# OPM/opm-autodiff

Measured on AMD Instinct MI355X. Metric: Newton iterations/sec, 1M-cell 3-phase black-oil (assembly + ILU0/BiCGStab solve + update), higher is better.
Workload: dtype f64

## Files before the change

include/opmhip.h:

```cpp
#ifndef OPMHIP_H
#define OPMHIP_H

#ifdef __cplusplus
extern "C" {
#endif

#define OPMHIP_ABI_VERSION 11

typedef struct opmhip_ctx opmhip_ctx;

typedef enum opmhip_status {
    OPMHIP_SUCCESS = 0,
    OPMHIP_ANALYSIS_FAILED = -1,
    OPMHIP_CREATE_PRECONDITIONER_FAILED = -2,
    OPMHIP_UNKNOWN_ERROR = -3,
    OPMHIP_INVALID_ARGUMENT = -4,
    OPMHIP_NOT_READY = -5,
    OPMHIP_DEVICE_ERROR = -6,
    OPMHIP_NO_DEVICE = -7
} opmhip_status;

typedef enum opmhip_reorder {
    OPMHIP_REORDER_LEVEL_SCHEDULING = 1,
    OPMHIP_REORDER_GRAPH_COLORING = 2,
// ... 16 lines not shown

typedef struct opmhip_config {
    int abi_version;
    int device_id;
    int verbosity;
    int maxit;
    double tolerance;
    double ilu_relaxation;
    int relax_mode;
    int reorder;
    int zero_diag_fix;
    int chain_length;
    int spmv_pipe_wgs;
    int preconditioner;
    int cpr_reuse_setup;
    int cpr_async_setup;
    int cpr_amg_ilu_levels;
    int cpr_gather_rows;
    int half_product;
    int pin_host_arrays;
    int fused_reductions;
} opmhip_config;

typedef struct opmhip_result {
    int iterations;
    int converged;
    double reduction;
    double conv_rate;
    double elapsed;
    double it;
    double t_copy;
    double t_factor;
    double t_solve;
    int num_colors;
    int reserved[3];
} opmhip_result;

typedef void (*opmhip_ms_apply_fn)(void* user, const double* h_x, double* h_y);
typedef struct opmhip_wells {
    int num_wells;
    const int* val_pointers;
    const int* Ccols;
    const int* Bcols;
    const double* Cnnzs;
    const double* Dnnzs;
    const double* Bnnzs;
    int num_ms_wells;
    opmhip_ms_apply_fn ms_apply;
    void* ms_user;
    int distributed;
} opmhip_wells;

#define OPMHIP_MS_WELLS_MAX_M 256
#define OPMHIP_MS_WELLS_MAX_KIB 32768
#define OPMHIP_MS_WELLS_TREE_MAX_SEGMENTS 1024
#define OPMHIP_MS_WELLS_DENSE 0
#define OPMHIP_MS_WELLS_TREE 1
#define OPMHIP_MS_WELLS_AUTO 2
typedef struct opmhip_ms_wells {
    int num_ms_wells;
    int dim, dim_wells;
    const int* Mb_pointers;
    const int* Brows;
    const int* block_pointers;
    const int* Bcols;
    const double* Bvals;
    const double* Cvals;
    const int* Dcol_pointers;
    const int* Drows;
    const double* Dvals;
    const int* Dnnz_pointers;
} opmhip_ms_wells;
int opmhip_set_ms_wells(opmhip_ctx* ctx, const opmhip_ms_wells* ms);
int opmhip_get_ms_wells_info(opmhip_ctx* ctx, int info[4]);
int opmhip_set_ms_wells_form(opmhip_ctx* ctx, int form);
int opmhip_get_ms_wells_form_info(opmhip_ctx* ctx, int info[6]);

void opmhip_default_config(opmhip_config* cfg);
int opmhip_create(const opmhip_config* cfg, opmhip_ctx** out);
void opmhip_destroy(opmhip_ctx* ctx);
const char* opmhip_last_error(const opmhip_ctx* ctx);
int opmhip_abi_version(void);
int opmhip_synchronize(opmhip_ctx* ctx);

int opmhip_set_pattern(opmhip_ctx* ctx, int Nb, int nnzb, const int* rows, const int* cols);
int opmhip_set_pattern_dd(opmhip_ctx* ctx, int Nb, int Nghost, int nnzb, const int* rows, const int* cols);

int opmhip_solve_system(opmhip_ctx* ctx, int N, int nnz, int dim, double* vals, const int* rows, const int* cols,
                        const double* b, const opmhip_wells* wells, opmhip_result* res);

int opmhip_get_result(opmhip_ctx* ctx, double* x);

int opmhip_wells_apply_residual(opmhip_ctx* ctx, const opmhip_wells* wells, const double* res_well);
int opmhip_add_well_contributions(opmhip_ctx* ctx, const opmhip_wells* wells);
int opmhip_get_rhs(opmhip_ctx* ctx, double* b);
int opmhip_wells_recover_solution(opmhip_ctx* ctx, const opmhip_wells* wells, const double* res_well, double* xw);

int opmhip_upload_system(opmhip_ctx* ctx, const double* vals, const double* b);
int opmhip_spmv(opmhip_ctx* ctx, const double* x, double* y);
int opmhip_ilu0_factor(opmhip_ctx* ctx, double* lu_out);
int opmhip_ilu0_apply(opmhip_ctx* ctx, const double* d, double* v);
int opmhip_preconditioned_product(opmhip_ctx* ctx, const double* d, double* t, double* z);
int opmhip_set_cpr_weights(opmhip_ctx* ctx, const double* weights);
int opmhip_cpr_recreate(opmhip_ctx* ctx);
int opmhip_get_cpr_weights(opmhip_ctx* ctx, double* weights);

int opmhip_cpr_apply(opmhip_ctx* ctx, const double* d, double* v);
int opmhip_get_ordering(opmhip_ctx* ctx, int* toOrder, int* fromOrder, int* rowsPerColor);
int opmhip_get_ordering_info(opmhip_ctx* ctx, int info[4]);
int opmhip_set_ilu_fillin_level(opmhip_ctx* ctx, int n);
int opmhip_get_ilu_info(opmhip_ctx* ctx, int info[4]);
int opmhip_get_ilu_factors(opmhip_ctx* ctx, int* toOrder, int* lrowptr, int* lcol, int* urowptr, int* ucol, double* L, double* U, double* invD);
int opmhip_get_product_form(opmhip_ctx* ctx, int info[4]);
int opmhip_get_split_assembly(opmhip_ctx* ctx, long long info[4], double* rest, double* matrix);
int opmhip_time_kernel(opmhip_ctx* ctx, int which, int reps, double* ms_per_launch);
int opmhip_cpr_levels(opmhip_ctx* ctx, int* n, int* nnz, int cap);

typedef struct opmhip_fluid {
    int num_pvt, num_sat;
    const double* pvtw;
    const double* density;
    const int* pvdg_ptr;
    const double* pvdg;
    const int* pvto_node_ptr;
    const double* pvto_rs;
    const int* pvto_row_ptr;
    const double* pvto;
    const int* swof_ptr;
    const double* swof;
    const int* sgof_ptr;
    const double* sgof;
    double rock_pref, rock_cr;
    const int* pvtg_node_ptr;
    const double* pvtg_pg;
    const int* pvtg_row_ptr;
    const double* pvtg;
    int num_rock;
    const int* rocktab_ptr;
    const double* rocktab;
    int pc_scaling;
} opmhip_fluid;

#define OPMHIP_SW_PO_SG 0
#define OPMHIP_SW_PO_RS 1
#define OPMHIP_SW_PG_RV 2

int opmhip_set_fluid(opmhip_ctx* ctx, const opmhip_fluid* fluid);

int opmhip_set_static(opmhip_ctx* ctx, const double* trans, const double* area, const double* thpres,
                      const double* poro, const double* volume, const double* depth, const int* pvtnum,
                      const int* satnum, const double* rsmax);

int opmhip_set_problem_extras(opmhip_ctx* ctx, const double* rvmax, const int* rocknum, const double* overburden);

int opmhip_set_composition_change_limits(opmhip_ctx* ctx, const double* drsdt, const int* drsdt_all_cells, const double* drvdt);

int opmhip_set_irreversible_compaction(opmhip_ctx* ctx, int enable);

int opmhip_set_vappars(opmhip_ctx* ctx, int enable, double vap1, double vap2);

int opmhip_set_water_compaction(opmhip_ctx* ctx, int num_tables, const int* num_pressure, const int* num_sw, const double* pressure,
                                const double* sw, const double* pv_mult, const double* trans_mult);
int opmhip_get_max_water_saturation(opmhip_ctx* ctx, double* max_water_saturation);

int opmhip_begin_time_step(opmhip_ctx* ctx, double dt);

// ... 204 lines not shown
```

opm-autodiff_amd/capi.py:

```python
import ctypes as C
import os
import re

import numpy as np

HERE = os.path.dirname(os.path.abspath(__file__))
LIB_PATH = os.environ.get("OPMHIP_LIB", os.path.join(HERE, "libopmhip.so"))
HEADER_PATH = os.path.join(os.path.dirname(HERE), "include", "opmhip.h")

SUCCESS = 0
ANALYSIS_FAILED, CREATE_PRECONDITIONER_FAILED, UNKNOWN_ERROR = -1, -2, -3
INVALID_ARGUMENT, NOT_READY, DEVICE_ERROR, NO_DEVICE = -4, -5, -6, -7
REORDER = {"level_scheduling": 1, "graph_coloring": 2, "graph_coloring_greedy": 3, "line_coloring": 4, "auto": 5, "distance2": 6}
RELAX = {"post_scale": 0, "in_sweep": 1}
PRECONDITIONER = {"ilu0": 0, "cpr_quasiimpes": 1, "cpr": 2, "cpr_trueimpes": 2}


class OpmHipError(RuntimeError):
    def __init__(self, code, msg):
        super().__init__("opmhip status %d: %s" % (code, msg))
        self.code = code


class Config(C.Structure):
# ... 258 lines not shown
    Mbp, blkp, nzp = [0], [0], [0]
    cat = {k: [] for k in ("Brows", "Bcols", "Bvals", "Cvals", "Dcolptr", "Drows", "Dvals")}
    for n, w in enumerate(wells):
        a = {k: np.asarray(w[k]).reshape(-1) for k in cat}
        Mb, nblk, nnz = len(a["Brows"]) - 1, len(a["Bcols"]), len(a["Dvals"])
        if Mb < 1:
            raise ValueError("multisegment well %d: Brows needs Mb + 1 >= 2 entries" % n)
        if a["Brows"][0] != 0 or a["Brows"][-1] != nblk or np.any(np.diff(a["Brows"]) < 0):
            raise ValueError("multisegment well %d: Brows must rise from 0 to the number of blocks (%d)" % (n, nblk))
        if len(a["Bvals"]) != 12 * nblk or len(a["Cvals"]) != 12 * nblk:
            raise ValueError("multisegment well %d: Bvals / Cvals need 12 values per block (%d blocks)" % (n, nblk))
        if len(a["Dcolptr"]) != 4 * Mb + 1:
            raise ValueError("multisegment well %d: Dcolptr needs 4 Mb + 1 = %d entries, has %d" % (n, 4 * Mb + 1, len(a["Dcolptr"])))
        if len(a["Drows"]) != nnz or a["Dcolptr"][0] != 0 or a["Dcolptr"][-1] != nnz or np.any(np.diff(a["Dcolptr"]) < 0):
            raise ValueError("multisegment well %d: Dcolptr must rise from 0 to len(Dvals) = len(Drows)" % n)
        for k in cat:
            cat[k].append(a[k])
        Mbp.append(Mbp[-1] + Mb)
        blkp.append(blkp[-1] + nblk)
        nzp.append(nzp[-1] + nnz)
    keep = [_i32(Mbp), _i32(np.concatenate(cat["Brows"])), _i32(blkp), _i32(np.concatenate(cat["Bcols"])), _f64(np.concatenate(cat["Bvals"])),
            _f64(np.concatenate(cat["Cvals"])), _i32(np.concatenate(cat["Dcolptr"])), _i32(np.concatenate(cat["Drows"])), _f64(np.concatenate(cat["Dvals"])), _i32(nzp)]
    return MsWells(len(wells), 3, 4, *[_ptr(k) for k in keep]), keep


def declared_symbols():
    with open(HEADER_PATH) as f:
        txt = re.sub(r"/\*.*?\*/", "", f.read(), flags=re.S)
    return sorted(set(re.findall(r"\b(opmhip_[a-z0-9_]+)\s*\(", txt)))


_lib = None


def lib():
    global _lib
    if _lib is None:
        if not os.path.exists(LIB_PATH):
            raise OpmHipError(NO_DEVICE, "libopmhip.so not built (%s); run `make -C %s` or "
                              "__graft_entry__.build() - there is no CPU fallback" % (LIB_PATH, HERE))
        L = C.CDLL(LIB_PATH)
        vp, ip, dp = C.c_void_p, C.c_void_p, C.c_void_p
        L.opmhip_abi_version.restype = C.c_int
        L.opmhip_default_config.argtypes = [C.POINTER(Config)]
        L.opmhip_default_config.restype = None
        L.opmhip_create.argtypes = [C.POINTER(Config), C.POINTER(vp)]
        L.opmhip_destroy.argtypes = [vp]
        L.opmhip_destroy.restype = None
        L.opmhip_last_error.argtypes = [vp]
        L.opmhip_last_error.restype = C.c_char_p
        L.opmhip_set_pattern.argtypes = [vp, C.c_int, C.c_int, ip, ip]
        L.opmhip_solve_system.argtypes = [vp, C.c_int, C.c_int, C.c_int, dp, ip, ip, dp, C.POINTER(Wells),
                                          C.POINTER(Result)]
        L.opmhip_get_result.argtypes = [vp, dp]
        L.opmhip_get_rhs.argtypes = [vp, dp]
        L.opmhip_add_well_contributions.argtypes = [vp, C.POINTER(Wells)]
        L.opmhip_wells_apply_residual.argtypes = [vp, C.POINTER(Wells), dp]
        L.opmhip_wells_recover_solution.argtypes = [vp, C.POINTER(Wells), dp, dp]
        L.opmhip_upload_system.argtypes = [vp, dp, dp]
        L.opmhip_spmv.argtypes = [vp, dp, dp]
        L.opmhip_ilu0_factor.argtypes = [vp, dp]
        L.opmhip_ilu0_apply.argtypes = [vp, dp, dp]
        L.opmhip_cpr_apply.argtypes = [vp, dp, dp]
        L.opmhip_preconditioned_product.argtypes = [vp, dp, dp, dp]
        L.opmhip_cpr_recreate.argtypes = [vp]
        L.opmhip_set_cpr_weights.argtypes = [vp, dp]
        L.opmhip_get_cpr_weights.argtypes = [vp, dp]
        L.opmhip_get_ordering.argtypes = [vp, ip, ip, ip]
        L.opmhip_get_ordering_info.argtypes = [vp, C.POINTER(C.c_int * 4)]
        L.opmhip_get_product_form.argtypes = [vp, C.POINTER(C.c_int * 4)]
        L.opmhip_get_split_assembly.argtypes = [vp, C.POINTER(C.c_longlong * 4), dp, dp]
        L.opmhip_set_ilu_fillin_level.argtypes = [vp, C.c_int]
        L.opmhip_get_ilu_info.argtypes = [vp, C.POINTER(C.c_int * 4)]
        L.opmhip_set_ms_wells.argtypes = [vp, C.POINTER(MsWells)]
        L.opmhip_get_ms_wells_info.argtypes = [vp, C.POINTER(C.c_int * 4)]
        L.opmhip_set_ms_wells_form.argtypes = [vp, C.c_int]
        L.opmhip_get_ms_wells_form_info.argtypes = [vp, C.POINTER(C.c_int * 6)]
        L.opmhip_get_ilu_factors.argtypes = [vp, ip, ip, ip, ip, ip, dp, dp, dp]
        L.opmhip_time_kernel.argtypes = [vp, C.c_int, C.c_int, C.POINTER(C.c_double)]
        L.opmhip_cpr_levels.argtypes = [vp, ip, ip, C.c_int]
        L.opmhip_profile_enable.argtypes = [vp, C.c_int]
        L.opmhip_profile_get.argtypes = [vp, C.c_int, C.POINTER(C.c_longlong), C.POINTER(C.c_double)]
        L.opmhip_synchronize.argtypes = [vp]
        L.opmhip_comm_info.argtypes = [vp, ip]
        L.opmhip_comm_selftest.argtypes = [vp, dp]
        L.opmhip_set_vfp_tables.argtypes = [vp, C.POINTER(VfpTables)]
        L.opmhip_vfp_probe.argtypes = [vp, C.c_int, C.c_int, C.c_int, dp, dp, dp, dp, dp, dp, dp]
        _lib = L
    return _lib


def _ptr(a):
    return None if a is None else a.ctypes.data_as(C.c_void_p)


def _f64(a):
    return None if a is None else np.ascontiguousarray(a, dtype=np.float64)


def _i32(a):
    return None if a is None else np.ascontiguousarray(a, dtype=np.int32)


def make_wells(w):
    if not w:
        return None, []
    nstd = int(w.get("numWells", 0))
    if nstd > 0:
        keep = [_i32(w["val_pointers"]), _i32(w["Ccols"]), _i32(w["Bcols"]), _f64(w["Cnnzs"]), _f64(w["Dnnzs"]), _f64(w["Bnnzs"])]
        s = Wells(nstd, *[_ptr(k) for k in keep])
    else:
        keep, s = [], Wells(0)
    nms = int(w.get("numMsWells", 0))
    if nms > 0:
        fn, n = w["ms_apply"], int(w["N"])

        def tramp(_user, hx, hy):
            fn(np.ctypeslib.as_array(hx, shape=(n,)), np.ctypeslib.as_array(hy, shape=(n,)))
        cb = MS_APPLY_FN(tramp)
        keep.append(cb)
        s.num_ms_wells, s.ms_apply = nms, cb
    s.distributed = int(w.get("distributed", 0))
    return s, keep


class HipSolver:

    def __init__(self, verbosity=0, maxit=200, tolerance=1e-2, device_id=0, ilu_relaxation=0.9,
                 relax_mode="post_scale", reorder=None, zero_diag_fix=True, chain_length=0, spmv_pipe_wgs=0,
                 preconditioner="ilu0", cpr_reuse_setup=3, cpr_async_setup=0, cpr_amg_ilu_levels=None, cpr_gather_rows=None, half_product=0, pin_host_arrays=0, fused_reductions=0,
                 ilu_fillin_level=0):
        L = lib()
        cfg = Config()
        L.opmhip_default_config(C.byref(cfg))
        cfg.verbosity, cfg.maxit, cfg.tolerance, cfg.device_id = verbosity, maxit, tolerance, device_id
        cfg.ilu_relaxation = ilu_relaxation
        cfg.relax_mode = RELAX[relax_mode]
        if reorder is not None:
            cfg.reorder = REORDER[reorder]
        cfg.zero_diag_fix = int(zero_diag_fix)
        cfg.chain_length = int(chain_length)
        cfg.spmv_pipe_wgs = int(spmv_pipe_wgs)
        cfg.preconditioner = PRECONDITIONER[preconditioner]
        if cpr_amg_ilu_levels is not None:
            cfg.cpr_amg_ilu_levels = int(cpr_amg_ilu_levels)
        if cpr_gather_rows is not None:
            cfg.cpr_gather_rows = int(cpr_gather_rows)
        cfg.half_product = int(half_product)
        cfg.fused_reductions = int(fused_reductions)
        self._pin = bool(pin_host_arrays)
        cfg.pin_host_arrays = int(pin_host_arrays)
        cfg.cpr_async_setup = int(cpr_async_setup)
        cfg.cpr_reuse_setup = int(cpr_reuse_setup)
        self._h = C.c_void_p()
        rc = L.opmhip_create(C.byref(cfg), C.byref(self._h))
        if rc != SUCCESS:
            raise OpmHipError(rc, L.opmhip_last_error(None).decode())
        self.Nb = self.nnzb = 0
        if ilu_fillin_level:
            self._check(L.opmhip_set_ilu_fillin_level(self._h, int(ilu_fillin_level)))

    def close(self):
        if getattr(self, "_h", None) and self._h.value:
            lib().opmhip_destroy(self._h)
            self._h = C.c_void_p()

# ... 120 lines not shown
    def ordering_info(self):
        info = (C.c_int * 4)()
        self._check(lib().opmhip_get_ordering_info(self._h, C.byref(info)))
        names = {v: k for k, v in REORDER.items()}
        return {"ilu_ordering": names[info[0]], "chain_length": int(info[1]), "colors": int(info[2]), "cpr_amg_ilu_levels": int(info[3])}

    def set_ilu_fillin_level(self, n):
        self._check(lib().opmhip_set_ilu_fillin_level(self._h, int(n)))

    def set_ms_wells(self, wells, form="dense"):
        ms, keep = make_ms_wells(wells)
        if ms:
            self._check(lib().opmhip_set_ms_wells_form(self._h, MS_WELLS_FORMS[form] if isinstance(form, str) else int(form)))
        self._check(lib().opmhip_set_ms_wells(self._h, C.byref(ms) if ms else None))

    def ms_wells_form_info(self):
        info = (C.c_int * 6)()
        self._check(lib().opmhip_get_ms_wells_form_info(self._h, C.byref(info)))
        names = {v: k for k, v in MS_WELLS_FORMS.items()}
        return {"form": names[int(info[0])], "dense": int(info[1]), "tree": int(info[2]), "tree_max_segments": int(info[3]), "tree_max_depth": int(info[4]),
                "tree_kib": int(info[5])}

    def ms_wells_info(self):
        info = (C.c_int * 4)()
        self._check(lib().opmhip_get_ms_wells_info(self._h, C.byref(info)))
        return {"wells": int(info[0]), "max_m": int(info[1]), "kib": int(info[2]), "factorisations": int(info[3])}

    def ilu_info(self):
        info = (C.c_int * 4)()
        self._check(lib().opmhip_get_ilu_info(self._h, C.byref(info)))
        return {"fill_level": int(info[0]), "nl": int(info[1]), "nu": int(info[2]), "levels": int(info[3])}

    def ilu_factors(self, values=True):
        inf = self.ilu_info()
        Nb, nl, nu = self.Nb, inf["nl"], inf["nu"]
        out = {"to": np.empty(Nb, np.int32), "lrowptr": np.empty(Nb + 1, np.int32), "lcol": np.empty(nl, np.int32),
               "urowptr": np.empty(Nb + 1, np.int32), "ucol": np.empty(nu, np.int32)}
        vals = [None, None, None]
        if values:
            vals = [np.empty((nl, 3, 3)), np.empty((nu, 3, 3)), np.empty((Nb, 3, 3))]
            out.update(L=vals[0], U=vals[1], invD=vals[2])
        self._check(lib().opmhip_get_ilu_factors(self._h, *[_ptr(out[k]) for k in ("to", "lrowptr", "lcol", "urowptr", "ucol")],
                                                 *[_ptr(v) for v in vals]))
        return out

    def product_form(self):
        info = (C.c_int * 4)()
        self._check(lib().opmhip_get_product_form(self._h, C.byref(info)))
        return {"half_product": bool(info[0]), "u_is_upper_a": bool(info[1]), "rest_blocks": int(info[2]), "rest_positions": int(info[3])}

    def split_assembly(self, rest=False, matrix=False):
        info = (C.c_longlong * 4)()
        r = np.empty((self.product_form()["rest_blocks"], 3, 3)) if rest else None
        m = np.empty(9 * self.nnzb) if matrix else None
        self._check(lib().opmhip_get_split_assembly(self._h, C.byref(info), _ptr(r), _ptr(m)))
        out = {"on": bool(info[0]), "stale": bool(info[1]), "assemblies": int(info[2]), "gathers": int(info[3])}
        if rest:
            out["rest"] = r
        if matrix:
            out["matrix"] = m
        return out

    PROF = ["spmv", "ilu_apply", "ilu_factor", "vector", "assemble", "iq_update", "convergence", "cpr_amg", "spmv_boundary",
            "halo", "allreduce", "cpr_gather"]

    def profile_enable(self, on=True):
        self._check(lib().opmhip_profile_enable(self._h, int(on)))

    def profile(self):
        out = {}
        for i, name in enumerate(self.PROF):
            n, ms = C.c_longlong(0), C.c_double(0.0)
            self._check(lib().opmhip_profile_get(self._h, i, C.byref(n), C.byref(ms)))
            out[name] = (n.value, ms.value)
        return out

    def cpr_levels(self):
        n, nnz = np.zeros(32, np.int32), np.zeros(32, np.int32)
        L = self._check(lib().opmhip_cpr_levels(self._h, _ptr(n), _ptr(nnz), 32))
        return [int(v) for v in n[:L]], [int(v) for v in nnz[:L]]

    def synchronize(self):
        self._check(lib().opmhip_synchronize(self._h))

    def comm_info(self):
        a = np.zeros(4, np.int32)
        self._check(lib().opmhip_comm_info(self._h, _ptr(a)))
        return {"nranks": int(a[0]), "rank": int(a[1]), "device": int(a[2]), "kind": ["none", "loopback", "rccl"][int(a[3])]}

    def comm_selftest(self):
        a = np.zeros(2)
        self._check(lib().opmhip_comm_selftest(self._h, _ptr(a)))
        return float(a[0]), float(a[1])

    def time_kernel(self, which, reps=20):
        ms = C.c_double()
        self._check(lib().opmhip_time_kernel(self._h, {"spmv": 0, "ilu_apply": 1, "ilu_factor": 2, "vector": 3, "stream_read": 4, "spmv_dot1": 5, "spmv_dot2": 6,
                                                              "rest_product": 7, "rest_product_dot2": 8, "ilu_apply_rowsums": 9}[which],
                                             reps, C.byref(ms)))
        return ms.value


def comm_unique_id():
    L = lib()
    if not getattr(L, "_asm_bound", False):
        _bind_assembly(L)
        L._asm_bound = True
    buf = C.create_string_buffer(128)
    rc = L.opmhip_comm_unique_id(buf)
    if rc != SUCCESS:
        raise OpmHipError(rc, "opmhip_comm_unique_id failed (librccl not loadable?)")
    return buf.raw


def _bind_assembly(L):
    vp = C.c_void_p
    L.opmhip_set_fluid.argtypes = [vp, vp]
    L.opmhip_set_static.argtypes = [vp] + [vp] * 9
    L.opmhip_set_state.argtypes = [vp, vp, vp]
    L.opmhip_get_state.argtypes = [vp, vp, vp]
    L.opmhip_advance_time_level.argtypes = [vp]
    L.opmhip_update_failed.argtypes = [vp]
    L.opmhip_end_time_step.argtypes = [vp, C.c_double]
    L.opmhip_set_drift_compensation.argtypes = [vp, C.c_int, C.c_double]
    L.opmhip_set_source.argtypes = [vp, vp, vp]
    L.opmhip_assemble.argtypes = [vp, C.c_double, C.c_int, vp, vp]
    L.opmhip_get_iq.argtypes = [vp, vp]
    L.opmhip_get_iq_cells.argtypes = [vp, C.c_int, vp, vp]
    L.opmhip_set_source_cells.argtypes = [vp, C.c_int, vp, vp, vp]
    L.opmhip_convergence.argtypes = [vp, C.c_double, C.c_double, vp]
    L.opmhip_update.argtypes = [vp, vp, C.c_double, C.POINTER(C.c_int)]
    L.opmhip_reservoir_averages.argtypes = [vp, vp]
    L.opmhip_set_pattern_dd.argtypes = [vp, C.c_int, C.c_int, C.c_int, vp, vp]
    L.opmhip_comm_unique_id.argtypes = [C.c_char_p]
    L.opmhip_comm_init_rccl.argtypes = [vp, C.c_int, C.c_int, C.c_char_p]
    L.opmhip_comm_init_loopback.argtypes = [vp, C.c_int, C.c_int, C.c_char_p]
    L.opmhip_set_halo.argtypes = [vp, C.c_longlong, C.c_int, vp, vp, vp, vp]
    L.opmhip_set_cell_global_ids.argtypes = [vp, vp]
    L.opmhip_fluid_probe.argtypes = [vp, C.c_int, C.c_int, C.c_int, vp, vp, vp, vp, vp]
    L.opmhip_set_problem_extras.argtypes = [vp, vp, vp, vp]
    L.opmhip_set_pcw.argtypes = [vp, vp]
    L.opmhip_set_endpoint_scaling.argtypes = [vp, vp]
    L.opmhip_set_composition_change_limits.argtypes = [vp, vp, vp, vp]
    L.opmhip_set_irreversible_compaction.argtypes = [vp, C.c_int]
    L.opmhip_begin_time_step.argtypes = [vp, C.c_double]
    L.opmhip_get_trackers.argtypes = [vp, vp, vp, vp, vp]
    L.opmhip_set_vappars.argtypes = [vp, C.c_int, C.c_double, C.c_double]
    L.opmhip_set_water_compaction.argtypes = [vp, C.c_int, vp, vp, vp, vp, vp, vp]
    L.opmhip_get_max_water_saturation.argtypes = [vp, vp]
    L.opmhip_relative_change.argtypes = [vp, C.POINTER(C.c_double)]
    L.opmhip_sat_end_points.argtypes = [vp, C.c_int, vp]
    L.opmhip_sat_probe.argtypes = [vp, C.c_int, vp, C.c_int, vp, vp, vp]
    L.opmhip_gas_probe.argtypes = [vp, C.c_int, C.c_int, vp, vp, vp]
    L.opmhip_iq_fields.argtypes = [vp]
    L.opmhip_set_hysteresis.argtypes = [vp, C.c_int, vp, vp]
    L.opmhip_get_hysteresis.argtypes = [vp, vp, vp, vp, vp]
    L.opmhip_set_hysteresis_params.argtypes = [vp, vp, vp]
    L.opmhip_set_aquifers.argtypes = [vp, C.POINTER(Aquifers)]
    L.opmhip_aquifers_begin_time_step.argtypes = [vp, C.c_double, C.c_double]
    L.opmhip_get_aquifers.argtypes = [vp, vp, vp, vp, vp]
    L.opmhip_get_aquifer_rates.argtypes = [vp, vp]
    L.opmhip_set_std_wells.argtypes = [vp, C.POINTER(StdWells)]
    L.opmhip_std_wells_begin_iteration.argtypes = [vp, C.c_int]
    L.opmhip_std_wells_apply_residual.argtypes = [vp]
    L.opmhip_std_wells_update.argtypes = [vp, C.c_double]
    L.opmhip_get_std_wells.argtypes = [vp, vp, vp, vp]
# ... 375 lines not shown
        n = getattr(self, "_nswperf", 0)
        if (pp is not None and pp.size != n) or (pr is not None and pr.size != 3 * n):
            raise ValueError("set_std_wells_perf_state: array lengths do not fit the %d perforations set" % n)
        self._check(lib().opmhip_set_std_wells_perf_state(self._h, _ptr(pp), _ptr(pr)))

    def std_wells_begin_iteration(self, iteration):
        self._check(lib().opmhip_std_wells_begin_iteration(self._h, int(iteration)))

    def std_wells_apply_residual(self):
        self._check(lib().opmhip_std_wells_apply_residual(self._h))

    def std_wells_update(self, relax=1.0):
        self._check(lib().opmhip_std_wells_update(self._h, float(relax)))

    def get_std_wells(self):
        n = getattr(self, "_nsw", 0)
        x, ctl, rw = np.zeros((n, 4)), np.zeros(n, np.int32), np.zeros((n, 4))
        self._check(lib().opmhip_get_std_wells(self._h, _ptr(x), _ptr(ctl), _ptr(rw)))
        return x, ctl, rw

    def set_std_wells_state(self, x=None, control=None, rate_target=None):
        x, control, rate_target = _f64(x), _i32(control), _f64(rate_target)
        n = getattr(self, "_nsw", 0)
        if (x is not None and x.size != 4 * n) or (control is not None and control.size != n) or (rate_target is not None and rate_target.size != n):
            raise ValueError("set_std_wells_state: array lengths do not fit the %d wells set" % n)
        self._check(lib().opmhip_set_std_wells_state(self._h, _ptr(x), _ptr(control), _ptr(rate_target)))

    def std_wells_blocks(self):
        n, p = getattr(self, "_nsw", 0), getattr(self, "_nswperf", 0)
        out = dict(head=np.zeros(p), D=np.zeros((n, 4, 4)), Dinv=np.zeros((n, 4, 4)), B=np.zeros((p, 4, 3)), C=np.zeros((p, 4, 3)), rates=np.zeros((p, 3, 5)),
                   xw=np.zeros((n, 4)))
        self._check(lib().opmhip_get_std_wells_blocks(self._h, *[_ptr(out[k]) for k in ("head", "D", "Dinv", "B", "C", "rates", "xw")]))
        return out

    def set_source(self, source, dsource=None):
        s, d = _f64(source), _f64(dsource)
        self._check(lib().opmhip_set_source(self._h, _ptr(s), _ptr(d)))

    def set_source_cells(self, cells, source, dsource=None):
        cl, s, d = _i32(cells), _f64(source), _f64(dsource)
        self._check(lib().opmhip_set_source_cells(self._h, len(cl), _ptr(cl), _ptr(s), _ptr(d)))

    def assemble(self, dt, iteration, fetch=True):
        jac = np.empty(9 * self.nnzb) if fetch else None
        res = np.empty(3 * self.Nb) if fetch else None
        self._check(lib().opmhip_assemble(self._h, dt, iteration, _ptr(jac), _ptr(res)))
        return jac, res

    def iq(self):
        nf = self._check(lib().opmhip_iq_fields(self._h))
        out = np.empty(self.Nloc * nf * 4)
        self._check(lib().opmhip_get_iq(self._h, _ptr(out)))
        return out.reshape(self.Nloc, nf, 4)

    def iq_cells(self, cells):
        cl = _i32(cells)
        nf = self._check(lib().opmhip_iq_fields(self._h))
        out = np.empty(len(cl) * nf * 4)
        self._check(lib().opmhip_get_iq_cells(self._h, len(cl), _ptr(cl), _ptr(out)))
        return out.reshape(len(cl), nf, 4)

    def convergence(self, dt, tol_cnv=1e-2):
        out = np.empty(17)
        self._check(lib().opmhip_convergence(self._h, dt, tol_cnv, _ptr(out)))
        return out

    def reservoir_averages(self):
        out = np.empty(5)
        self._check(lib().opmhip_reservoir_averages(self._h, _ptr(out)))
        return out

    def solve_jacobian_system(self, wells=None):
        res = Result()
        ws, keep = make_wells(wells)
        self._check(lib().opmhip_solve_system(self._h, 3 * self.Nb, 9 * self.nnzb, 3, None, None, None, None,
                                              C.byref(ws) if ws else None, C.byref(res)))
        return res

    def update(self, dx=None, relax=1.0):
        dx = _f64(dx)
        n = C.c_int(0)
        self._check(lib().opmhip_update(self._h, _ptr(dx), relax, C.byref(n)))
        return n.value
```

opm-autodiff_amd/csrc/assemble.hip:

```cpp
#include <hip/hip_runtime.h>

#include <cfloat>

#include "device_blocks.hpp"
#include "fluid_device.hpp"

namespace opmhip {

template <class E> __device__ __forceinline__ E wc_eval(const int* __restrict__ d, const double* __restrict__ data, int voff, const E& xv, const E& yv) {
    const int ns = d[1];
    const double* xs = data + d[2];
    const double* ys = data + d[3];
    const int i = seg_right(xs, d[0], val(xv));
    const E alpha = (xv - xs[i]) / (xs[i + 1] - xs[i]);
    const double* v1 = data + voff + (size_t)i * ns;
    const double* v2 = v1 + ns;
    const int j1 = seg_right(ys, ns, val(yv)), j2 = j1;
    const E beta1 = (yv - ys[j1]) / (ys[j1 + 1] - ys[j1]);
    const E beta2 = (yv - ys[j2]) / (ys[j2 + 1] - ys[j2]);
    const E s1 = v1[j1] * (1.0 - beta1) + v1[j1 + 1] * beta1;
    const E s2 = v2[j2] * (1.0 - beta2) + v2[j2 + 1] * beta2;
    return s1 * (1.0 - alpha) + s2 * alpha;
}
template <class E, class DP> __device__ __forceinline__ void cap_pressures(const TablesT<DP>& T, int sr, const E& Sw, const E& Sg, E pC[3]) {
// ... 432 lines not shown
    iq_update_body<EXT>(c0, Nb, T, C, pv, meaning, iq);
}
template <>
__global__ __launch_bounds__(256) IQ_OCC void k_iq_update<false>(int c0, int Nb, Tables T, CellStatic C, const double* __restrict__ pv,
                                                                 const unsigned char* __restrict__ meaning, double* __restrict__ iq) {
    iq_update_body<false>(c0, Nb, T, C, pv, meaning, iq);
}

template <class DP, bool EXT>
__device__ __forceinline__ void newton_update_cell(const TablesT<DP>& T, const CellStatic& C, int c, const double* __restrict__ dx, double relax,
                                                   double* __restrict__ pv, unsigned char* __restrict__ meaning,
                                                   unsigned char* __restrict__ wasSwitched, double* __restrict__ iq,
                                                   int* __restrict__ nswitched) {
    const double dpMaxRel = 0.3, dsMax = 0.2, oscThreshold = 1e-5;
    double x[3] = {pv[(size_t)c * 3], pv[(size_t)c * 3 + 1], pv[(size_t)c * 3 + 2]};
    double u[3] = {dx[(size_t)c * 3], dx[(size_t)c * 3 + 1], dx[(size_t)c * 3 + 2]};
    if (relax != 1.0) { u[0] *= relax; u[1] *= relax; u[2] *= relax; }
    int mng = meaning[c];
    const double deltaSw = u[0];
    double deltaSo = -deltaSw, deltaSg = 0.0;
    if (mng == OPMHIP_SW_PO_SG) { deltaSg = u[2]; deltaSo -= deltaSg; }
    double maxSatDelta = fmax(fabs(deltaSg), fabs(deltaSo));
    maxSatDelta = fmax(maxSatDelta, fabs(deltaSw));
    double satAlpha = 1.0;
    if (maxSatDelta > dsMax) satAlpha = dsMax / maxSatDelta;
    double nx[3];
    {
        double delta = u[0] * satAlpha;
        nx[0] = x[0] - delta;
        delta = u[1];
        if (fabs(delta) > dpMaxRel * x[1]) delta = (delta < 0.0 ? -1.0 : 1.0) * dpMaxRel * x[1];
        nx[1] = x[1] - delta;
        delta = u[2];
        if (mng == OPMHIP_SW_PO_SG) delta *= satAlpha;
        else if (delta > x[2]) delta = x[2];
        nx[2] = x[2] - delta;
    }
    x[0] = nx[0]; x[1] = nx[1]; x[2] = nx[2];
    const int pr = C.pvtnum ? C.pvtnum[c] : 0, sr = C.satnum ? C.satnum[c] : 0;
    const double RsMax = C.rsmax ? C.rsmax[c] : DBL_MAX / 2.0;
    const bool wet = EXT && T.pvt(pr).wg_n > 0;
    const double eps = wasSwitched[c] ? oscThreshold : 0.0;
    bool sw = false;
    const bool vap = EXT && C.maxso;
    auto vap_f = [&](double So_, double par) { return vap ? vappars_factor<double>(So_, emax(So_, C.maxso[c]), par) : 1.0; };
    if (x[0] >= 1.0) {
        x[0] = 1.0; x[2] = 0.0;
        sw = mng != OPMHIP_SW_PO_SG;
        mng = OPMHIP_SW_PO_SG;
    } else if (mng == OPMHIP_SW_PO_SG) {
        const double So = 1.0 - x[0] - x[2];
        if (x[2] < -eps && So > 0.0) {
            mng = OPMHIP_SW_PO_RS;
            x[2] = emin(RsMax, rs_sat_value(T, pr, x[1]) * vap_f(So, C.vap2));
            sw = true;
        } else if (EXT && wet && So < -eps && x[2] > 0.0) {
            double pC[3];
            cell_cap_pressures<DP, EXT>(T, C, c, sr, x[0], x[2], pC);
            const double pg = x[1] + (pC[GAS] - pC[OIL]);
            const double RvMax = C.rvmax ? C.rvmax[c] : DBL_MAX / 2.0;
            mng = OPMHIP_SW_PG_RV;
            x[1] = pg;
            x[2] = emin(RvMax, rv_sat_value(T, pr, pg) * vap_f(So, C.vap1));
            sw = true;
        }
    } else if (!EXT || mng == OPMHIP_SW_PO_RS) {
        const double RsSat = rs_sat_value(T, pr, x[1]) * vap_f(1.0 - x[0], C.vap2);
        if (x[2] > emin(RsMax, RsSat * (1.0 + eps))) { mng = OPMHIP_SW_PO_SG; x[2] = 0.0; sw = true; }
    } else {
        const double RvMax = C.rvmax ? C.rvmax[c] : DBL_MAX / 2.0;
        const double RvSat = rv_sat_value(T, pr, x[1]) * vap_f(0.0, C.vap1);
        if (x[2] > emin(RvMax, RvSat * (1.0 + eps))) {
            double pC[3];
            cell_cap_pressures<DP, EXT>(T, C, c, sr, x[0], 1.0 - x[0], pC);
            mng = OPMHIP_SW_PO_SG;
            x[1] = x[1] + (pC[OIL] - pC[GAS]);
            x[2] = 1.0 - x[0];
            sw = true;
        }
    }
    wasSwitched[c] = sw ? 1 : 0;
    meaning[c] = (unsigned char)mng;
    pv[(size_t)c * 3] = x[0]; pv[(size_t)c * 3 + 1] = x[1]; pv[(size_t)c * 3 + 2] = x[2];
    if (sw) atomicAdd(nswitched, 1);
    Iq<Ad> q;
    update_iq<Ad, DP, EXT>(T, C, c, x, mng, q);
    store_iq<EXT>(iq, C.ncell, c, q);
    store_invb(C.invb, c, q);
}
template <bool EXT>
__device__ __forceinline__ void newton_update_body(int Nb, const Tables& T, const CellStatic& C, const double* __restrict__ dx, double relax,
                                                   double* __restrict__ pv, unsigned char* __restrict__ meaning,
                                                   unsigned char* __restrict__ wasSwitched, double* __restrict__ iq,
                                                   int* __restrict__ nswitched) {
    __shared__ double s_tab[TAB_LDS_DBL];
    const bool inLds = tables_to_lds(T, s_tab);
    const int c = blockIdx.x * blockDim.x + threadIdx.x;
    if (c >= Nb) return;
    if (inLds) newton_update_cell<LdsTab, EXT>(lds_tables(T, s_tab), C, c, dx, relax, pv, meaning, wasSwitched, iq, nswitched);
    else newton_update_cell<GlobalTab, EXT>(T, C, c, dx, relax, pv, meaning, wasSwitched, iq, nswitched);
}
template <bool EXT>
__global__ __launch_bounds__(256) void k_newton_update(int Nb, Tables T, CellStatic C, const double* __restrict__ dx, double relax,
                                                       double* __restrict__ pv, unsigned char* __restrict__ meaning,
                                                       unsigned char* __restrict__ wasSwitched, double* __restrict__ iq,
                                                       int* __restrict__ nswitched) {
    newton_update_body<EXT>(Nb, T, C, dx, relax, pv, meaning, wasSwitched, iq, nswitched);
}
template <>
__global__ __launch_bounds__(256) IQ_OCC void k_newton_update<false>(int Nb, Tables T, CellStatic C, const double* __restrict__ dx, double relax,
                                                                     double* __restrict__ pv, unsigned char* __restrict__ meaning,
                                                                     unsigned char* __restrict__ wasSwitched, double* __restrict__ iq,
                                                                     int* __restrict__ nswitched) {
    newton_update_body<false>(Nb, T, C, dx, relax, pv, meaning, wasSwitched, iq, nswitched);
}

__global__ __launch_bounds__(256) void k_fluid_probe(Tables T, int pr, int sr, int n, const double* __restrict__ p,
                                                     const double* __restrict__ rs, const double* __restrict__ sw,
                                                     const double* __restrict__ sg, double* __restrict__ out) {
    const int i = blockIdx.x * blockDim.x + threadIdx.x;
    if (i >= n) return;
    const PvtRegionDesc& D = T.pvt(pr);
    const SatRegionDesc& Sd = T.sat(sr);
    const GlobalTab B = T.dbl;
    double* o = out + (size_t)i * 8;
    const double pi = p[i], rsi = rs[i];
    o[0] = pvt_invBw(T, D, pi);
    const bool wetg = D.wg_n > 0;
    o[1] = wetg ? tab1<double, GlobalTab>(B + D.wg_xs, B + D.wgs_invB, D.wg_n, pi) : tab1<double, GlobalTab>(B + D.gas_p, B + D.gas_invB, D.gas_n, pi);
    const double RsSat = rs_sat_value(T, pr, pi);
    o[3] = RsSat;
    o[2] = pvt_invBo(T, pr, D, pi, rsi);
    if (rsi >= RsSat) o[6] = o[2] / tab1<double, GlobalTab>(B + D.sat_p, B + D.sat_invBMu, D.sat_n, pi);
    else o[6] = o[2] / tab2<double, GlobalTab>(T, D, D.o_invBMu, rsi, pi);
    const double Swco = B[Sd.swco];
    o[4] = pwlin<double, GlobalTab>(B + Sd.sw_x, B + Sd.pcow, Sd.nw, sw[i]);
    o[5] = pwlin<double, GlobalTab>(B + Sd.so_x, B + Sd.pcgo, Sd.ng, 1.0 - Swco - sg[i]);
    o[7] = o[1] / (wetg ? tab1<double, GlobalTab>(B + D.wg_xs, B + D.wgs_invBMu, D.wg_n, pi) : tab1<double, GlobalTab>(B + D.gas_p, B + D.gas_invBMu, D.gas_n, pi));
}
__global__ __launch_bounds__(256) void k_gas_probe(Tables T, int pr, int n, const double* __restrict__ p, const double* __restrict__ rv,
                                                   double* __restrict__ out) {
    const int i = blockIdx.x * blockDim.x + threadIdx.x;
    if (i >= n) return;
    const PvtRegionDesc& D = T.pvt(pr);
    const GlobalTab B = T.dbl;
    double* o = out + (size_t)i * 3;
    const double pi = p[i], rvi = rv[i];
    o[0] = pvt_invBg(T, pr, D, pi, rvi);
    if (D.wg_n > 0) {
        const double RvSat = rv_sat_value(T, pr, pi);
        o[2] = RvSat;
        if (rvi >= RvSat) o[1] = o[0] / tab1<double, GlobalTab>(B + D.wg_xs, B + D.wgs_invBMu, D.wg_n, pi);
        else o[1] = o[0] / tab2wg<double, GlobalTab>(T, D, D.wg_invBMu, pi, rvi);
    } else {
        o[1] = o[0] / tab1<double, GlobalTab>(B + D.gas_p, B + D.gas_invBMu, D.gas_n, pi);
        o[2] = 0.0;
    }
}
int launch_gas_probe(opmhip_ctx* c, int pr, int n, const double* d_in, double* d_out) {
    hipLaunchKernelGGL(k_gas_probe, dim3((n + 255) / 256), dim3(256), 0, c->stream, tables_of(c), pr, n, d_in, d_in + n, d_out);
    return OPMHIP_SUCCESS;
}
__global__ __launch_bounds__(256) void k_sat_probe(Tables T, int sr, int cfg, const double* __restrict__ eps, int n, const double* __restrict__ sw,
                                                   const double* __restrict__ sg, double* __restrict__ out) {
    const int i = blockIdx.x * blockDim.x + threadIdx.x;
    if (i >= n) return;
    const SatRegionDesc& Sd = T.sat(sr);
// ... 299 lines not shown
    double a[10];
    for (int i = 0; i < 10; ++i) a[i] = (i >= 3 && i < 6) ? -DBL_MAX : 0.0;
    if (c < Nb) {
        const double pvValue = C.poro[c] * C.volume[c];
        const int comp[3] = {EQ_WATER, EQ_OIL, EQ_GAS};
        for (int ph = 0; ph < 3; ++ph) {
            const int e = comp[ph];
            a[6 + e] = 1.0 / C.invb[(size_t)c * 3 + ph];
            const double R2 = resid[(size_t)c * 3 + e];
            a[e] = R2;
            a[3 + e] = fabs(R2) / pvValue;
        }
        a[9] = pvValue;
    }
    const int lane = threadIdx.x & 63, wv = threadIdx.x >> 6;
    for (int i = 0; i < 10; ++i) {
        double v = a[i];
        for (int o = 32; o > 0; o >>= 1) {
            const double w = __shfl_down(v, o, 64);
            v = (i >= 3 && i < 6) ? fmax(v, w) : v + w;
        }
        if (lane == 0) sh[i][wv] = v;
    }
    __syncthreads();
    if (threadIdx.x < 10) {
        const int i = threadIdx.x;
        double v = sh[i][0];
        for (int w = 1; w < 4; ++w) v = (i >= 3 && i < 6) ? fmax(v, sh[i][w]) : v + sh[i][w];
        part[(size_t)blockIdx.x * 10 + i] = v;
    }
}
__global__ void k_conv_pack(const double* __restrict__ out, double* __restrict__ red) {
    if (threadIdx.x < 3) { red[threadIdx.x] = out[threadIdx.x]; red[3 + threadIdx.x] = out[6 + threadIdx.x]; red[8 + threadIdx.x] = out[3 + threadIdx.x]; }
    if (threadIdx.x == 0) red[6] = out[9];
}
__global__ void k_conv_unpack(const double* __restrict__ red, double global_cells, double* __restrict__ out) {
    if (threadIdx.x < 3) { out[threadIdx.x] = red[threadIdx.x]; out[6 + threadIdx.x] = red[3 + threadIdx.x] / global_cells; out[3 + threadIdx.x] = red[8 + threadIdx.x]; }
    if (threadIdx.x == 0) out[9] = red[6];
}
__global__ __launch_bounds__(256) void k_conv_final1(int nblocks, int Nb, const double* __restrict__ part, double* __restrict__ out) {
    __shared__ double sh[10][256];
    double a[10];
    for (int i = 0; i < 10; ++i) a[i] = (i >= 3 && i < 6) ? -DBL_MAX : 0.0;
    for (int b = threadIdx.x; b < nblocks; b += 256)
        for (int i = 0; i < 10; ++i) {
            const double v = part[(size_t)b * 10 + i];
            a[i] = (i >= 3 && i < 6) ? fmax(a[i], v) : a[i] + v;
        }
    for (int i = 0; i < 10; ++i) sh[i][threadIdx.x] = a[i];
    __syncthreads();
    for (int o = 128; o > 0; o >>= 1) {
        if ((int)threadIdx.x < o)
            for (int i = 0; i < 10; ++i) {
                const double v = sh[i][threadIdx.x + o];
                sh[i][threadIdx.x] = (i >= 3 && i < 6) ? fmax(sh[i][threadIdx.x], v) : sh[i][threadIdx.x] + v;
            }
        __syncthreads();
    }
    if (threadIdx.x < 10) {
        double v = sh[threadIdx.x][0];
        if (threadIdx.x >= 6 && threadIdx.x < 9 && Nb > 0) v /= (double)Nb;
        out[threadIdx.x] = v;
    }
}
__global__ __launch_bounds__(256) void k_conv_pass2(int Nb, CellStatic C, const double* __restrict__ resid, const double* __restrict__ out1,
                                                    double dt, double tol_cnv, double* __restrict__ part) {
    __shared__ double sh[4];
    const int c = blockIdx.x * blockDim.x + threadIdx.x;
    double v = 0.0;
    if (c < Nb) {
        const double pvValue = C.poro[c] * C.volume[c];
        bool violated = false;
        for (int e = 0; e < 3; ++e) {
            const double CNV = resid[(size_t)c * 3 + e] * dt * out1[6 + e] / pvValue;
            violated = violated || (fabs(CNV) > tol_cnv);
        }
        if (violated) v = pvValue;
    }
    for (int o = 32; o > 0; o >>= 1) v += __shfl_down(v, o, 64);
    if ((threadIdx.x & 63) == 0) sh[threadIdx.x >> 6] = v;
    __syncthreads();
    if (threadIdx.x == 0) part[blockIdx.x] = sh[0] + sh[1] + sh[2] + sh[3];
}
__global__ __launch_bounds__(256) void k_conv_final2(int nblocks, const double* __restrict__ part, double* __restrict__ out) {
    __shared__ double sh[256];
    double a = 0.0;
    for (int b = threadIdx.x; b < nblocks; b += 256) a += part[b];
    sh[threadIdx.x] = a;
    __syncthreads();
    for (int o = 128; o > 0; o >>= 1) {
        if ((int)threadIdx.x < o) sh[threadIdx.x] += sh[threadIdx.x + o];
        __syncthreads();
    }
    if (threadIdx.x == 0) out[10] = sh[0];
}

constexpr int RESV_SUMS = 8;
template <bool EXT>
__global__ __launch_bounds__(256) void k_resv_avg_part(int Nb, int ncell, const double* __restrict__ iq, const double* __restrict__ volume,
                                                       double* __restrict__ part) {
    __shared__ double sh[RESV_SUMS][4];
    double a[RESV_SUMS];
    for (int i = 0; i < RESV_SUMS; ++i) a[i] = 0.0;
    for (size_t c = (size_t)blockIdx.x * 256 + threadIdx.x; c < (size_t)Nb; c += (size_t)gridDim.x * 256) {
        const int ci = (int)c;
        const double pv_cell = volume[ci] * iq_at(iq, ncell, Lay<EXT>::F_PORO, ci)[0];
        double hydrocarbon = 1.0;
        hydrocarbon -= iq_at(iq, ncell, F_S + WATER, ci)[0];
        const double po = iq_at(iq, ncell, F_P + OIL, ci)[0], Rs = iq_at(iq, ncell, F_RS, ci)[0];
        const double Rv = EXT ? iq_at(iq, ncell, Lay<EXT>::F_RV, ci)[0] : 0.0;
        const double hpv = pv_cell * hydrocarbon;
        if (hpv > 0.0) { a[0] += hpv; a[1] += po * hpv; a[2] += Rs * hpv; a[3] += Rv * hpv; }
        if (pv_cell > 0.0) { a[4] += pv_cell; a[5] += po * pv_cell; a[6] += Rs * pv_cell; a[7] += Rv * pv_cell; }
    }
    const int lane = threadIdx.x & 63, wv = threadIdx.x >> 6;
    for (int i = 0; i < RESV_SUMS; ++i) {
        double v = a[i];
        for (int o = 32; o > 0; o >>= 1) v += __shfl_down(v, o, 64);
        if (lane == 0) sh[i][wv] = v;
    }
    __syncthreads();
    if (threadIdx.x < RESV_SUMS) {
        const int i = threadIdx.x;
        part[(size_t)blockIdx.x * RESV_SUMS + i] = ((sh[i][0] + sh[i][1]) + sh[i][2]) + sh[i][3];
    }
}
__global__ __launch_bounds__(RESV_FINAL_THREADS) void k_resv_avg_final(int nblocks, const double* __restrict__ part, double* __restrict__ out) {
    __shared__ double sh[RESV_SUMS][RESV_FINAL_THREADS];
    double a[RESV_SUMS];
    for (int i = 0; i < RESV_SUMS; ++i) a[i] = 0.0;
    for (int b = threadIdx.x; b < nblocks; b += RESV_FINAL_THREADS)
        for (int i = 0; i < RESV_SUMS; ++i) a[i] += part[(size_t)b * RESV_SUMS + i];
    for (int i = 0; i < RESV_SUMS; ++i) sh[i][threadIdx.x] = a[i];
    __syncthreads();
    for (int o = RESV_FINAL_THREADS / 2; o > 0; o >>= 1) {
        if ((int)threadIdx.x < o)
            for (int i = 0; i < RESV_SUMS; ++i) sh[i][threadIdx.x] += sh[i][threadIdx.x + o];
        __syncthreads();
    }
    if (threadIdx.x == 0) {
        const double hpv_sum = sh[0][0], pv_sum = sh[4][0];
        const int k = hpv_sum > 0.0 ? 0 : 4;
        const double w = sh[k][0];
        const bool ok = hpv_sum > 0.0 || pv_sum > 0.0;
        out[0] = ok ? sh[k + 1][0] / w : 0.0;
        out[1] = ok ? sh[k + 2][0] / w : 0.0;
        out[2] = ok ? sh[k + 3][0] / w : 0.0;
        out[3] = w;
        out[4] = k == 0 ? 1.0 : 0.0;
        out[5] = pv_sum;
    }
}

__global__ void k_drift_update(int n, const double* __restrict__ resid, double dt, double* __restrict__ drift) {
    const int e = blockIdx.x * blockDim.x + threadIdx.x;
    if (e < n) drift[e] = resid[e] * dt;
}
template <bool EXT>
__global__ __launch_bounds__(256) void k_last_rs_rv(int N, const int* __restrict__ pvtnum, const int* __restrict__ drsdt_all, const double* __restrict__ iq,
                                                    double* __restrict__ lastRs, double* __restrict__ lastRv) {
    const int c = blockIdx.x * blockDim.x + threadIdx.x;
    if (c >= N) return;
    if (lastRs) {
        const int pr = pvtnum ? pvtnum[c] : 0;
        const double Sg = iq_at(iq, N, F_S + GAS, c)[0];
        lastRs[c] = (drsdt_all[pr] || Sg > 1e-7) ? iq_at(iq, N, F_RS, c)[0] : INFINITY;
    }
    if (EXT && lastRv) lastRv[c] = iq_at(iq, N, Lay<EXT>::F_RV, c)[0];
}
__global__ __launch_bounds__(256) void k_set_limits(int N, double dt, const int* __restrict__ pvtnum, const double* __restrict__ drsdt, const double* __restrict__ drvdt,
                                                    const double* __restrict__ lastRs, const double* __restrict__ lastRv, double* __restrict__ rsmax, double* __restrict__ rvmax) {
    const int c = blockIdx.x * blockDim.x + threadIdx.x;
    if (c >= N) return;
    const int pr = pvtnum ? pvtnum[c] : 0;
    if (drsdt) rsmax[c] = (drsdt[pr] < 0.0) ? DBL_MAX / 2.0 : lastRs[c] + drsdt[pr] * dt;
    if (drvdt) rvmax[c] = (drvdt[pr] < 0.0) ? DBL_MAX / 2.0 : lastRv[c] + drvdt[pr] * dt;
}
// ... 143 lines not shown
    hipLaunchKernelGGL(k_aquifer_begin, dim3((Q.nc + 63) / 64), dim3(64), 0, c->stream, Q.nc, c->pat.Nloc, Q.d_pos, c->asmb.d_iq, Q.d_pprev);
}
void launch_aquifer_apply(opmhip_ctx* c) {
    const AquifersDev& Q = c->asmb.aq;
    hipLaunchKernelGGL(k_aquifer_apply, dim3((Q.nd + 63) / 64), dim3(64), 0, c->stream, Q.nd, c->pat.Nloc, aquifer_arrays(Q), Q.d_cpos, Q.d_cptr, Q.d_cconn,
                       c->asmb.d_iq, c->asmb.d_depth, c->asmb.d_source, c->asmb.d_dsource, Q.d_save, Q.d_q);
}
void launch_aquifer_restore(opmhip_ctx* c) {
    const AquifersDev& Q = c->asmb.aq;
    hipLaunchKernelGGL(k_aquifer_restore, dim3((Q.nd + 63) / 64), dim3(64), 0, c->stream, Q.nd, Q.d_cpos, Q.d_save, c->asmb.d_source, c->asmb.d_dsource);
}
void launch_aquifer_end(opmhip_ctx* c, double dt) {
    const AquifersDev& Q = c->asmb.aq;
    hipLaunchKernelGGL(k_aquifer_end, dim3((Q.num + 63) / 64), dim3(64), 0, c->stream, Q.num, dt, Q.d_ptr, Q.d_par, Q.d_q, Q.d_state);
}

__global__ void k_cellvec_to_internal_u8(int Nb, const int* __restrict__ fromOrder, const unsigned char* __restrict__ nat, unsigned char* __restrict__ internal) {
    const int p = blockIdx.x * blockDim.x + threadIdx.x;
    if (p < Nb) internal[p] = nat[fromOrder[p]];
}
__global__ void k_cellvec_to_natural_u8(int Nb, const int* __restrict__ toOrder, const unsigned char* __restrict__ internal, unsigned char* __restrict__ nat) {
    const int i = blockIdx.x * blockDim.x + threadIdx.x;
    if (i < Nb) nat[i] = internal[toOrder[i]];
}
__global__ void k_iq_to_natural(int Nb, int IQS, const int* __restrict__ toOrder, const double* __restrict__ internal, double* __restrict__ nat) {
    const size_t e = (size_t)blockIdx.x * blockDim.x + threadIdx.x;
    if (e >= (size_t)Nb * IQS) return;
    const int i = (int)(e / IQS), q = (int)(e % IQS);
    nat[e] = internal[((size_t)(q >> 2) * Nb + toOrder[i]) * 4 + (q & 3)];
}
__global__ void k_iq_gather(int n, int IQS, int Nb, const int* __restrict__ pos, const double* __restrict__ internal, double* __restrict__ out) {
    const size_t e = (size_t)blockIdx.x * blockDim.x + threadIdx.x;
    if (e >= (size_t)n * IQS) return;
    const int i = (int)(e / IQS), q = (int)(e % IQS);
    out[e] = internal[((size_t)(q >> 2) * Nb + pos[i]) * 4 + (q & 3)];
}
__global__ void k_source_scatter(int n, const int* __restrict__ pos, const double* __restrict__ src, const double* __restrict__ dsrc,
                                 double* __restrict__ source, double* __restrict__ dsource) {
    const int e = blockIdx.x * blockDim.x + threadIdx.x;
    if (e >= n * 12) return;
    const int i = e / 12, q = e % 12;
    if (q < 3) source[(size_t)pos[i] * 3 + q] = src[(size_t)i * 3 + q];
    else if (dsrc) dsource[(size_t)pos[i] * 9 + (q - 3)] = dsrc[(size_t)i * 9 + (q - 3)];
}
__global__ void k_unpermute_blocks(int nnzb, const int* __restrict__ nnzMap, const double* __restrict__ internal, double* __restrict__ nat) {
    const size_t e = (size_t)blockIdx.x * blockDim.x + threadIdx.x;
    if (e >= (size_t)nnzb * BB) return;
    const int k = (int)(e / BB), q = (int)(e % BB);
    nat[(size_t)nnzMap[k] * BB + q] = internal[e];
}

static inline int cdiv(size_t a, size_t b) { return (int)((a + b - 1) / b); }
static CellStatic cells_of(const opmhip_ctx* c) {
    return CellStatic{c->asmb.d_poro, c->asmb.d_volume, c->asmb.d_depth, c->asmb.d_rsmax, c->asmb.d_pvtnum, c->asmb.d_satnum,
                      c->asmb.d_rvmax, c->asmb.d_overburden, c->asmb.d_rocknum, c->asmb.d_pcw, c->asmb.d_minpo, c->asmb.d_maxso, c->asmb.vap1, c->asmb.vap2,
                      c->asmb.d_maxsw, c->asmb.d_sw0, c->asmb.d_wcdesc, c->asmb.d_wcdata, c->asmb.d_eps, c->asmb.epscfg,
                      c->asmb.d_hyst, c->asmb.d_imbnum, c->asmb.d_eps_imb, c->asmb.hyst_model, c->asmb.d_invb, c->pat.Nloc};
}
void launch_hyst_update(opmhip_ctx* c, const double* d_sw_ow, const double* d_sw_go) {
    const int N = c->pat.Nloc;
    hipLaunchKernelGGL(k_hyst_update, dim3((N + 255) / 256), dim3(256), 0, c->stream, N, tables_of(c), cells_of(c), c->asmb.d_iq, c->asmb.d_hyst, d_sw_ow, d_sw_go);
}
#define OPMHIP_LAYOUT(c, call_base, call_ext) do { if ((c)->asmb.ext) { call_ext; } else { call_base; } } while (0)

void launch_iq_update(opmhip_ctx* c) {
    const int Nb = c->pat.Nloc;
    const int ps = prof_begin(c, PROF_IQ_UPDATE);
    OPMHIP_LAYOUT(c,
        hipLaunchKernelGGL(k_iq_update<false>, dim3(cdiv(Nb, 256)), dim3(256), 0, c->stream, 0, Nb, tables_of(c), cells_of(c), c->asmb.d_pv, c->asmb.d_meaning, c->asmb.d_iq),
        hipLaunchKernelGGL(k_iq_update<true>, dim3(cdiv(Nb, 256)), dim3(256), 0, c->stream, 0, Nb, tables_of(c), cells_of(c), c->asmb.d_pv, c->asmb.d_meaning, c->asmb.d_iq));
    prof_end(c, ps);
}
int launch_ghost_refresh(opmhip_ctx* c) {
    if (c->comm.nranks <= 1 || c->pat.Nghost == 0) return OPMHIP_SUCCESS;
    int rc;
    if ((rc = comm_halo_f64(c, c->asmb.d_pv, 3))) return rc;
    if ((rc = comm_halo_u8(c, c->asmb.d_meaning))) return rc;
    const int Nb = c->pat.Nb, Nloc = c->pat.Nloc;
    OPMHIP_LAYOUT(c,
        hipLaunchKernelGGL(k_iq_update<false>, dim3(cdiv(Nloc - Nb, 256)), dim3(256), 0, c->stream, Nb, Nloc, tables_of(c), cells_of(c), c->asmb.d_pv, c->asmb.d_meaning, c->asmb.d_iq),
        hipLaunchKernelGGL(k_iq_update<true>, dim3(cdiv(Nloc - Nb, 256)), dim3(256), 0, c->stream, Nb, Nloc, tables_of(c), cells_of(c), c->asmb.d_pv, c->asmb.d_meaning, c->asmb.d_iq));
    return OPMHIP_SUCCESS;
}
void launch_newton_update(opmhip_ctx* c, const double* d_dx, double relax) {
    const int Nb = c->pat.Nb;
    (void)hipMemsetAsync(c->asmb.d_nswitched, 0, sizeof(int), c->stream);
    const int ps = prof_begin(c, PROF_IQ_UPDATE);
    OPMHIP_LAYOUT(c,
        hipLaunchKernelGGL(k_newton_update<false>, dim3(cdiv(Nb, 256)), dim3(256), 0, c->stream, Nb, tables_of(c), cells_of(c), d_dx, relax, c->asmb.d_pv,
                           c->asmb.d_meaning, c->asmb.d_wasSwitched, c->asmb.d_iq, c->asmb.d_nswitched),
        hipLaunchKernelGGL(k_newton_update<true>, dim3(cdiv(Nb, 256)), dim3(256), 0, c->stream, Nb, tables_of(c), cells_of(c), d_dx, relax, c->asmb.d_pv,
                           c->asmb.d_meaning, c->asmb.d_wasSwitched, c->asmb.d_iq, c->asmb.d_nswitched));
    prof_end(c, ps);
}
void launch_assemble(opmhip_ctx* c, double dt, int iteration) {
    EntryStatic ES{c->asmb.d_trans, c->asmb.d_area, c->asmb.d_thpres};
    const int ps = prof_begin(c, PROF_ASSEMBLE);
    const double* drift = c->asmb.drift_enabled ? c->asmb.d_drift : (const double*)nullptr;
    const int grid = c->asmb.nsched;
    if (iteration == 0 && c->asmb.storage_frozen) iteration = 1;
    const bool split = c->split_asm && c->asmb.split_ok && !c->wells.sw.ma.on;
#define OPMHIP_ASM_LAUNCH(EXT, SPL, WET)                                                                                                                                   \
    hipLaunchKernelGGL((k_assemble<EXT, SPL>), dim3(grid), dim3(ASM_THREADS), 0, c->stream, c->asmb.nsched, reinterpret_cast<const int4*>(c->asmb.d_asm_sched),                \
                       reinterpret_cast<const int2*>(c->asmb.d_asm_desc), WET, ES, cells_of(c), c->asmb.d_iq, c->asmb.d_storageOld, c->asmb.d_source, c->asmb.d_dsource, drift, \
                       c->asmb.max_compensation, dt, iteration, SPL ? c->d_R : c->d_A, c->d_b, c->d_U, c->pat.d_rrowptr, c->pat.d_urowptr)
    if (split) { OPMHIP_LAYOUT(c, OPMHIP_ASM_LAUNCH(false, true, 0), OPMHIP_ASM_LAUNCH(true, true, c->asmb.wet_gas ? 1 : 0)); }
    else { OPMHIP_LAYOUT(c, OPMHIP_ASM_LAUNCH(false, false, 0), OPMHIP_ASM_LAUNCH(true, false, c->asmb.wet_gas ? 1 : 0)); }
#undef OPMHIP_ASM_LAUNCH
    c->A_stale = split;
    if (split) c->split_assemblies++;
    prof_end(c, ps);
}
void launch_last_rs_rv(opmhip_ctx* c) {
    const AsmDev& A = c->asmb;
    const int N = c->pat.Nloc;
    OPMHIP_LAYOUT(c, hipLaunchKernelGGL(k_last_rs_rv<false>, dim3((N + 255) / 256), dim3(256), 0, c->stream, N, A.d_pvtnum, A.d_drsdt_all, A.d_iq, A.drsdt_on ? A.d_lastRs : nullptr, (double*)nullptr),
                  hipLaunchKernelGGL(k_last_rs_rv<true>, dim3((N + 255) / 256), dim3(256), 0, c->stream, N, A.d_pvtnum, A.d_drsdt_all, A.d_iq, A.drsdt_on ? A.d_lastRs : nullptr, A.drvdt_on ? A.d_lastRv : nullptr));
}
void launch_set_limits(opmhip_ctx* c, double dt) {
    const AsmDev& A = c->asmb;
    const int N = c->pat.Nloc;
    hipLaunchKernelGGL(k_set_limits, dim3((N + 255) / 256), dim3(256), 0, c->stream, N, dt, A.d_pvtnum, A.drsdt_on ? A.d_drsdt : nullptr, A.drvdt_on ? A.d_drvdt : nullptr,
                       A.d_lastRs, A.d_lastRv, A.d_rsmax, A.d_rvmax);
}
void launch_min_pressure(opmhip_ctx* c, bool init) {
    const int N = c->pat.Nloc;
    hipLaunchKernelGGL(k_min_pressure, dim3((N + 255) / 256), dim3(256), 0, c->stream, N, init ? 1 : 0, c->asmb.d_iq, c->asmb.d_minpo);
}
void launch_max_oil_saturation(opmhip_ctx* c, bool init) {
    const int N = c->pat.Nloc;
    hipLaunchKernelGGL(k_max_oil_saturation, dim3((N + 255) / 256), dim3(256), 0, c->stream, N, init ? 1 : 0, c->asmb.d_iq, c->asmb.d_maxso);
}
void launch_max_water_saturation(opmhip_ctx* c, bool init) {
    const Pattern& P = c->pat;
    const int N = P.Nloc;
    if (!init && N > 1) hipLaunchKernelGGL(k_copy_entry, dim3(1), dim3(1), 0, c->stream, c->asmb.d_maxsw, P.toOrder[1], P.toOrder[0]);
    hipLaunchKernelGGL(k_max_water_saturation, dim3((N + 255) / 256), dim3(256), 0, c->stream, N, init ? 1 : 0, c->asmb.d_iq, c->asmb.d_maxsw, c->asmb.d_sw0);
}
void launch_storage_old(opmhip_ctx* c) {
    const AsmDev& A = c->asmb;
    const int Nb = c->pat.Nb, N = c->pat.Nloc;
    OPMHIP_LAYOUT(c, hipLaunchKernelGGL(k_storage_old<false>, dim3((Nb + 255) / 256), dim3(256), 0, c->stream, Nb, N, 0, A.d_iq, A.d_storageOld),
                  hipLaunchKernelGGL(k_storage_old<true>, dim3((Nb + 255) / 256), dim3(256), 0, c->stream, Nb, N, A.wet_gas ? 1 : 0, A.d_iq, A.d_storageOld));
}

constexpr int RC_PARTS = 256;
__global__ __launch_bounds__(256) void k_relative_change_part(int Nb, const double* __restrict__ pv, const unsigned char* __restrict__ mg,
                                                              const double* __restrict__ pvOld, const unsigned char* __restrict__ mgOld,
                                                              double* __restrict__ part) {
    __shared__ double sd[256], sn[256];
    double delta = 0.0, denom = 0.0;
    for (int c = blockIdx.x * 256 + threadIdx.x; c < Nb; c += RC_PARTS * 256) {
        const double* a = &pv[(size_t)c * 3];
        const double* b = &pvOld[(size_t)c * 3];
        double sN[3] = {0.0, 0.0, 0.0}, sO[3] = {0.0, 0.0, 0.0};
        double oilN = 1.0, oilO = 1.0;
        sN[WATER] = a[0]; oilN -= sN[WATER];
        if (mg[c] == OPMHIP_SW_PO_SG) { sN[GAS] = a[2]; oilN -= sN[GAS]; }
        sN[OIL] = oilN;
        const double tmp = a[1] - b[1];
        double d = tmp * tmp, q = a[1] * a[1];
        sO[WATER] = b[0]; oilO -= sO[WATER];
        if (mgOld[c] == OPMHIP_SW_PO_SG) { sO[GAS] = b[2]; oilO -= sO[GAS]; }
        sO[OIL] = oilO;
#pragma unroll
        for (int ph = 0; ph < 3; ++ph) {
            const double t = sN[ph] - sO[ph];
            d += t * t;
            q += sN[ph] * sN[ph];
        }
        delta += d;
        denom += q;
    }
    sd[threadIdx.x] = delta; sn[threadIdx.x] = denom;
    __syncthreads();
    for (int h = 128; h > 0; h >>= 1) {
        if ((int)threadIdx.x < h) { sd[threadIdx.x] += sd[threadIdx.x + h]; sn[threadIdx.x] += sn[threadIdx.x + h]; }
        __syncthreads();
    }
    if (threadIdx.x == 0) { part[blockIdx.x] = sd[0]; part[RC_PARTS + blockIdx.x] = sn[0]; }
}
__global__ __launch_bounds__(64) void k_relative_change_final(const double* __restrict__ part, double* __restrict__ out) {
    if (threadIdx.x != 0) return;
    double d = 0.0, q = 0.0;
    for (int i = 0; i < RC_PARTS; ++i) { d += part[i]; q += part[RC_PARTS + i]; }
    out[0] = d; out[1] = q;
}
int launch_relative_change(opmhip_ctx* c) {
    const AsmDev& A = c->asmb;
    double* part = A.d_rc;
    double* out = A.d_rc + 2 * RC_PARTS;
    hipLaunchKernelGGL(k_relative_change_part, dim3(RC_PARTS), dim3(256), 0, c->stream, c->pat.Nb, A.d_pv, A.d_meaning, A.d_pv_prev, A.d_meaning_prev, part);
    hipLaunchKernelGGL(k_relative_change_final, dim3(1), dim3(64), 0, c->stream, part, out);
    if (c->comm.nranks > 1) return comm_allreduce(c, out, 2, 0);
    return OPMHIP_SUCCESS;
}

int launch_convergence(opmhip_ctx* c, double dt, double tol_cnv) {
    const int Nb = c->pat.Nb, nb = cdiv(Nb, 256);
    const int ps = prof_begin(c, PROF_CONVERGENCE);
    hipLaunchKernelGGL(k_conv_pass1, dim3(nb), dim3(256), 0, c->stream, Nb, cells_of(c), c->d_b, c->asmb.d_conv_part);
    const bool dd = c->comm.nranks > 1;
    hipLaunchKernelGGL(k_conv_final1, dim3(1), dim3(256), 0, c->stream, nb, dd ? 0 : Nb, c->asmb.d_conv_part, c->asmb.d_conv_out);
    if (dd) {
        hipLaunchKernelGGL(k_conv_pack, dim3(1), dim3(64), 0, c->stream, c->asmb.d_conv_out, c->comm.d_red);
        int rc;
        if ((rc = comm_allreduce(c, c->comm.d_red, 7, 0))) return rc;
        if ((rc = comm_allreduce(c, c->comm.d_red + 8, 3, 1))) return rc;
        hipLaunchKernelGGL(k_conv_unpack, dim3(1), dim3(64), 0, c->stream, c->comm.d_red, (double)c->comm.global_cells, c->asmb.d_conv_out);
    }
    hipLaunchKernelGGL(k_conv_pass2, dim3(nb), dim3(256), 0, c->stream, Nb, cells_of(c), c->d_b, c->asmb.d_conv_out, dt, tol_cnv, c->asmb.d_conv_part);
    hipLaunchKernelGGL(k_conv_final2, dim3(1), dim3(256), 0, c->stream, nb, c->asmb.d_conv_part, c->asmb.d_conv_out);
    if (dd) {
        const int rc = comm_allreduce(c, c->asmb.d_conv_out + 10, 1, 0);
        if (rc) return rc;
    }
    prof_end(c, ps);
    return OPMHIP_SUCCESS;
}
double* resv_avg_kernels(opmhip_ctx* c) {
    const int Nb = c->pat.Nb, nb = cdiv(Nb, 256) < RESV_MAX_PARTS ? cdiv(Nb, 256) : RESV_MAX_PARTS;
    double* part = c->asmb.d_resv;
    double* avg = part + (size_t)RESV_MAX_PARTS * RESV_SUMS;
    OPMHIP_LAYOUT(c,
        hipLaunchKernelGGL(k_resv_avg_part<false>, dim3(nb), dim3(256), 0, c->stream, Nb, c->pat.Nloc, c->asmb.d_iq, c->asmb.d_volume, part),
        hipLaunchKernelGGL(k_resv_avg_part<true>, dim3(nb), dim3(256), 0, c->stream, Nb, c->pat.Nloc, c->asmb.d_iq, c->asmb.d_volume, part));
    hipLaunchKernelGGL(k_resv_avg_final, dim3(1), dim3(RESV_FINAL_THREADS), 0, c->stream, nb, part, avg);
    return avg;
}
void launch_reservoir_averages(opmhip_ctx* c) {
    const int ps = prof_begin(c, PROF_ASSEMBLE);
    resv_avg_kernels(c);
    prof_end(c, ps);
}
void launch_u8_to_internal(opmhip_ctx* c, const unsigned char* nat, unsigned char* internal) {
    hipLaunchKernelGGL(k_cellvec_to_internal_u8, dim3(cdiv(c->pat.Nloc, 256)), dim3(256), 0, c->stream, c->pat.Nloc, c->pat.d_fromOrder, nat, internal);
}
void launch_u8_to_natural(opmhip_ctx* c, const unsigned char* internal, unsigned char* nat) {
    hipLaunchKernelGGL(k_cellvec_to_natural_u8, dim3(cdiv(c->pat.Nloc, 256)), dim3(256), 0, c->stream, c->pat.Nloc, c->pat.d_toOrder, internal, nat);
}
void launch_iq_to_natural(opmhip_ctx* c, double* d_nat) {
    const size_t n = (size_t)c->pat.Nloc * iq_doubles_per_cell(c);
    hipLaunchKernelGGL(k_iq_to_natural, dim3(cdiv(n, 256)), dim3(256), 0, c->stream, c->pat.Nloc, iq_doubles_per_cell(c), c->pat.d_toOrder, c->asmb.d_iq, d_nat);
}
void launch_iq_gather(opmhip_ctx* c, int n, const int* d_pos, double* d_out) {
    const int IQS = iq_doubles_per_cell(c);
    hipLaunchKernelGGL(k_iq_gather, dim3(cdiv((size_t)n * IQS, 256)), dim3(256), 0, c->stream, n, IQS, c->pat.Nloc, d_pos, c->asmb.d_iq, d_out);
}
void launch_source_scatter(opmhip_ctx* c, int n, const int* d_pos, const double* d_src, const double* d_dsrc) {
    hipLaunchKernelGGL(k_source_scatter, dim3(cdiv((size_t)n * 12, 256)), dim3(256), 0, c->stream, n, d_pos, d_src, d_dsrc, c->asmb.d_source, c->asmb.d_dsource);
}
void launch_unpermute_blocks(opmhip_ctx* c, const double* internal, double* nat) {
    const size_t n = (size_t)c->pat.nnzb * BB;
    hipLaunchKernelGGL(k_unpermute_blocks, dim3(cdiv(n, 256)), dim3(256), 0, c->stream, c->pat.nnzb, c->pat.d_nnzMap, internal, nat);
}
int iq_doubles_per_cell(const opmhip_ctx* c) { return c->asmb.ext ? Lay<true>::IQS : Lay<false>::IQS; }

}
```

opm-autodiff_amd/csrc/capi.cpp:

```cpp
#include <cstdlib>
#include <chrono>
#include <unordered_map>
#include <algorithm>
#include <climits>
#include <cstring>
#include <new>
#include <optional>

#include "internal.hpp"
#include "ms_wells_setup.hpp"

using namespace opmhip;

namespace {
thread_local std::string g_err = "";

double now() {
    return std::chrono::duration<double>(std::chrono::steady_clock::now().time_since_epoch()).count();
}

int alloc_system(opmhip_ctx* c) {
    const Pattern& P = c->pat;
    const size_t n = (size_t)P.Nloc * BS;
    int rc;
    constexpr size_t SLACK = 2 * BB;
    if ((rc = dev_alloc(c, &c->d_A, (size_t)P.nnzb * BB + SLACK))) return rc;
    if ((rc = dev_alloc(c, &c->d_L, (size_t)P.nl * BB + SLACK))) return rc;
    if ((rc = dev_alloc(c, &c->d_U, (size_t)P.nu * BB + SLACK))) return rc;
    OPMHIP_HIP(c, hipMemsetAsync(c->d_A + (size_t)P.nnzb * BB, 0, SLACK * sizeof(double), c->stream));
    const size_t l0 = P.fillLevel > 0 ? 0 : (size_t)P.nl * BB, u0 = P.fillLevel > 0 ? 0 : (size_t)P.nu * BB;
    OPMHIP_HIP(c, hipMemsetAsync(c->d_L + l0, 0, ((size_t)P.nl * BB + SLACK - l0) * sizeof(double), c->stream));
    OPMHIP_HIP(c, hipMemsetAsync(c->d_U + u0, 0, ((size_t)P.nu * BB + SLACK - u0) * sizeof(double), c->stream));
    if ((rc = dev_alloc(c, &c->d_invD, (size_t)P.Nb * BB))) return rc;
    c->half_product = half_product_wanted(c);
    if (c->half_product) {
        if ((rc = dev_alloc(c, &c->d_R, (size_t)P.nr * BB + SLACK))) return rc;
        OPMHIP_HIP(c, hipMemsetAsync(c->d_R, 0, ((size_t)P.nr * BB + SLACK) * sizeof(double), c->stream));
        if ((rc = dev_alloc(c, &c->d_usum, n))) return rc;
        OPMHIP_HIP(c, hipMemsetAsync(c->d_usum, 0, n * sizeof(double), c->stream));
    }
    c->split_asm = split_asm_wanted(c);
    c->A_stale = false;
    double** vecs[] = {&c->d_b, &c->d_x, &c->d_r, &c->d_rw, &c->d_p, &c->d_v, &c->d_s, &c->d_t, &c->d_pw, &c->d_vu, &c->d_stageV};
    for (double** v : vecs) {
        if ((rc = dev_alloc(c, v, n))) return rc;
        OPMHIP_HIP(c, hipMemsetAsync(*v, 0, n * sizeof(double), c->stream));
    }
    if ((rc = dev_alloc(c, &c->d_stageA, (size_t)P.nnzb * BB))) return rc;
    if ((rc = dev_alloc(c, &c->d_scal, (size_t)SC_COUNT))) return rc;
    OPMHIP_HIP(c, hipMemsetAsync(c->d_scal, 0, SC_COUNT * sizeof(double), c->stream));
    const int vb = (int)((n + 2047) / 2048);
    c->npart = std::max(std::max(P.tiles.ntiles(), P.tiles.nsched), vb) + 1;
    if ((rc = dev_alloc(c, &c->d_part, (size_t)3 * c->npart))) return rc;
    OPMHIP_HIP(c, hipMemsetAsync(c->d_part, 0, (size_t)3 * c->npart * sizeof(double), c->stream));
    if ((rc = dev_alloc(c, &c->d_part2, (size_t)1024))) return rc;
    OPMHIP_HIP(c, hipMemsetAsync(c->d_part2, 0, 1024 * sizeof(double), c->stream));
    if (!c->h_pinned) OPMHIP_HIP(c, hipHostMalloc((void**)&c->h_pinned, SC_COUNT * sizeof(double)));
    if (!c->h_ring) {
    OPMHIP_HIP(c, hipHostMalloc((void**)&c->h_ring, opmhip_ctx::RB_SLOTS * opmhip_ctx::RB_DOUBLES * sizeof(double), hipHostMallocMapped));
    OPMHIP_HIP(c, hipHostGetDevicePointer((void**)&c->d_ring, c->h_ring, 0));
    std::memset(c->h_ring, 0, opmhip_ctx::RB_SLOTS * opmhip_ctx::RB_DOUBLES * sizeof(double));
    }
    c->d_done = c->d_scal + SC_ZERO;
    OPMHIP_HIP(c, hipStreamSynchronize(c->stream));
    return OPMHIP_SUCCESS;
}

static bool no_standard_wells(const opmhip_ctx* c, const opmhip_wells* w) {
    return !w || (w->num_wells <= 0 && !(w->distributed != 0 && c->comm.nranks > 1));
}

static int upload_wells_local(opmhip_ctx* c, const opmhip_wells* w) {
    WellsDev& W = c->wells;
    if (W.sw.num > 0 && w->num_wells > 0)
        return fail(c, OPMHIP_INVALID_ARGUMENT, "wells: a host list of %d standard wells while a device-resident list of %d is set (opmhip_set_std_wells): the operator would be "
                    "applied twice", w->num_wells, W.sw.num);
    if (w->num_ms_wells > 0) {
        if (!w->ms_apply) return fail(c, OPMHIP_INVALID_ARGUMENT, "wells: num_ms_wells = %d but ms_apply == NULL", w->num_ms_wells);
        if (c->comm.nranks > 1) return fail(c, OPMHIP_INVALID_ARGUMENT, "wells: multisegment wells through the host callback are not supported in decomposed runs");
        if (W.ms.num > 0)
            return fail(c, OPMHIP_INVALID_ARGUMENT, "wells: num_ms_wells = %d with a callback while a device-resident list of %d multisegment wells is set "
                        "(opmhip_set_ms_wells): the operator would be applied twice", w->num_ms_wells, W.ms.num);
        const size_t bytes = (size_t)c->pat.Nb * BS * sizeof(double);
        if (!W.h_x) OPMHIP_HIP(c, hipHostMalloc((void**)&W.h_x, bytes));
        if (!W.h_y) OPMHIP_HIP(c, hipHostMalloc((void**)&W.h_y, bytes));
        W.num_ms = w->num_ms_wells;
        W.ms_apply = w->ms_apply;
        W.ms_user = w->ms_user;
    }
    if (w->num_wells <= 0) return OPMHIP_SUCCESS;
    if (!w->val_pointers || !w->Dnnzs) return fail(c, OPMHIP_INVALID_ARGUMENT, "wells: null array");
    const int nw = w->num_wells, np = w->val_pointers[nw];
    if (np < 0) return fail(c, OPMHIP_INVALID_ARGUMENT, "wells: bad val_pointers");
    if (np > 0 && (!w->Ccols || !w->Bcols || !w->Cnnzs || !w->Bnnzs)) return fail(c, OPMHIP_INVALID_ARGUMENT, "wells: null array");
    std::vector<int> cc(np), bc(np);
// ... 162 lines not shown
        launch_vec_to_internal(c, c->d_stageV, c->d_b);
    }
    if (vals && c->cfg.zero_diag_fix) launch_zero_diag_fix(c);
    OPMHIP_HIP(c, hipGetLastError());
    if (vals) c->system_loaded = true;
    return OPMHIP_SUCCESS;
}

int vec_in(opmhip_ctx* c, const double* h, double* d_internal) {
    OPMHIP_HIP(c, hipMemcpyAsync(c->d_stageV, h, (size_t)c->pat.Nb * BS * sizeof(double), hipMemcpyHostToDevice, c->stream));
    launch_vec_to_internal(c, c->d_stageV, d_internal);
    return OPMHIP_SUCCESS;
}
int vec_out(opmhip_ctx* c, const double* d_internal, double* h) {
    launch_vec_to_natural(c, d_internal, c->d_stageV);
    OPMHIP_HIP(c, hipMemcpyAsync(h, c->d_stageV, (size_t)c->pat.Nb * BS * sizeof(double), hipMemcpyDeviceToHost, c->stream));
    OPMHIP_HIP(c, hipStreamSynchronize(c->stream));
    return OPMHIP_SUCCESS;
}

template <class F>
int guarded(opmhip_ctx* c, F&& f) {
    try {
        return f();
    } catch (const std::bad_alloc&) {
        return fail(c, OPMHIP_UNKNOWN_ERROR, "out of host memory");
    } catch (const std::exception& e) {
        return fail(c, OPMHIP_UNKNOWN_ERROR, "exception: %s", e.what());
    } catch (...) {
        return fail(c, OPMHIP_UNKNOWN_ERROR, "unknown exception");
    }
}
}

extern "C" {

int opmhip_abi_version(void) { return OPMHIP_ABI_VERSION; }

void opmhip_default_config(opmhip_config* cfg) {
    if (!cfg) return;
    std::memset(cfg, 0, sizeof *cfg);
    cfg->abi_version = OPMHIP_ABI_VERSION;
    cfg->device_id = 0;
    cfg->verbosity = 0;
    cfg->maxit = 200;
    cfg->tolerance = 1e-2;
    cfg->ilu_relaxation = 0.9;
    cfg->relax_mode = OPMHIP_RELAX_POST_SCALE;
    cfg->reorder = OPMHIP_REORDER_AUTO;
    cfg->cpr_amg_ilu_levels = -1;
    cfg->zero_diag_fix = 1;
    cfg->cpr_reuse_setup = 3;
}

int opmhip_create(const opmhip_config* cfg, opmhip_ctx** out) {
    if (!out) { g_err = "opmhip_create: out == NULL"; return OPMHIP_INVALID_ARGUMENT; }
    *out = nullptr;
    if (!cfg || cfg->abi_version != OPMHIP_ABI_VERSION) { g_err = "opmhip_create: config missing or ABI version mismatch"; return OPMHIP_INVALID_ARGUMENT; }
    if (cfg->maxit < 1 || !(cfg->tolerance > 0.0)) { g_err = "opmhip_create: maxit/tolerance out of range"; return OPMHIP_INVALID_ARGUMENT; }
    if (cfg->preconditioner < OPMHIP_PRECOND_ILU0 || cfg->preconditioner > OPMHIP_PRECOND_CPR_TRUEIMPES) { g_err = "opmhip_create: unknown preconditioner"; return OPMHIP_INVALID_ARGUMENT; }
    if (cfg->chain_length < 0) { g_err = "opmhip_create: chain_length < 0"; return OPMHIP_INVALID_ARGUMENT; }
    if (cfg->cpr_reuse_setup < 0 || cfg->cpr_reuse_setup > 3) { g_err = "opmhip_create: cpr_reuse_setup must be 0 .. 3"; return OPMHIP_INVALID_ARGUMENT; }
    if (cfg->cpr_async_setup < 0 || cfg->cpr_async_setup > 1) { g_err = "opmhip_create: cpr_async_setup must be 0 or 1"; return OPMHIP_INVALID_ARGUMENT; }
    if (cfg->fused_reductions < 0 || cfg->fused_reductions > 1) { g_err = "opmhip_create: fused_reductions must be 0 or 1"; return OPMHIP_INVALID_ARGUMENT; }
    if (cfg->fused_reductions && cfg->tolerance < 1e-6) { g_err = "opmhip_create: fused_reductions needs tolerance >= 1e-6 (the recurred residual norm cannot resolve less than sqrt(eps) |r_0|)"; return OPMHIP_INVALID_ARGUMENT; }
    if (cfg->pin_host_arrays < 0 || cfg->pin_host_arrays > 1) { g_err = "opmhip_create: pin_host_arrays must be 0 or 1"; return OPMHIP_INVALID_ARGUMENT; }
    int ndev = 0;
    hipError_t e = hipGetDeviceCount(&ndev);
    if (e != hipSuccess || ndev <= 0) {
        g_err = std::string("opmhip_create: no HIP device visible (") + hipGetErrorString(e) + "); libopmhip has no CPU fallback";
        return OPMHIP_NO_DEVICE;
    }
    if (cfg->device_id < 0 || cfg->device_id >= ndev) { g_err = "opmhip_create: device_id out of range"; return OPMHIP_INVALID_ARGUMENT; }
    opmhip_ctx* c = new (std::nothrow) opmhip_ctx();
    if (!c) { g_err = "opmhip_create: out of memory"; return OPMHIP_UNKNOWN_ERROR; }
    c->cfg = *cfg;
    c->device = cfg->device_id;
    if ((e = hipSetDevice(c->device)) != hipSuccess || (e = hipStreamCreateWithFlags(&c->stream, hipStreamNonBlocking)) != hipSuccess ||
        (e = hipEventCreate(&c->ev0)) != hipSuccess || (e = hipEventCreate(&c->ev1)) != hipSuccess) {
        g_err = std::string("opmhip_create: ") + hipGetErrorString(e);
        delete c;
        return OPMHIP_DEVICE_ERROR;
    }
    *out = c;
    return OPMHIP_SUCCESS;
}

void opmhip_destroy(opmhip_ctx* c) {
    if (!c) return;
    (void)hipSetDevice(c->device);
    if (c->stream) (void)hipStreamSynchronize(c->stream);
    cpr_shutdown(c);
    comm_release(c);
    for (const auto& r : c->pinned)
        if (r.bytes) (void)hipHostUnregister(const_cast<void*>(r.p));
    for (void* p : c->allocs) (void)hipFree(p);
    if (c->h_pinned) (void)hipHostFree(c->h_pinned);
    if (c->wells.h_x) (void)hipHostFree(c->wells.h_x);
    if (c->wells.h_y) (void)hipHostFree(c->wells.h_y);
    if (c->wells.ms.h_flag) (void)hipHostFree(c->wells.ms.h_flag);
    if (c->h_ring) (void)hipHostFree(c->h_ring);
    if (c->asmb.aq.h_step) (void)hipHostFree(c->asmb.aq.h_step);
    if (c->asmb.aq.ev_step) (void)hipEventDestroy(c->asmb.aq.ev_step);
    if (c->ev0) (void)hipEventDestroy(c->ev0);
    if (c->ev1) (void)hipEventDestroy(c->ev1);
    for (hipEvent_t e : c->prof.ev) (void)hipEventDestroy(e);
    if (c->stream) (void)hipStreamDestroy(c->stream);
    delete c;
}

const char* opmhip_last_error(const opmhip_ctx* c) { return c ? c->err.c_str() : g_err.c_str(); }

int opmhip_synchronize(opmhip_ctx* c) {
    if (!c) return OPMHIP_INVALID_ARGUMENT;
    OPMHIP_HIP(c, hipSetDevice(c->device));
    OPMHIP_HIP(c, hipStreamSynchronize(c->stream));
    return OPMHIP_SUCCESS;
}

int opmhip_set_pattern(opmhip_ctx* c, int Nb, int nnzb, const int* rows, const int* cols) {
    return opmhip_set_pattern_dd(c, Nb, 0, nnzb, rows, cols);
}

int opmhip_set_pattern_dd(opmhip_ctx* c, int Nb, int Nghost, int nnzb, const int* rows, const int* cols) {
    if (!c) return OPMHIP_INVALID_ARGUMENT;
    return guarded(c, [&]() -> int {
        if (c->pattern_set) return fail(c, OPMHIP_NOT_READY, "set_pattern: the pattern of a context is immutable (linalg/ISTLSolverEbos.hpp:216-219)");
        OPMHIP_HIP(c, hipSetDevice(c->device));
        int rc = build_pattern(c, Nb, Nghost, nnzb, rows, cols);
        if (rc) return rc;
        for (int i = 0; i < Nb; ++i)
            if (rows[i + 1] - rows[i] > TILE_CAP_BLOCKS)
                return fail(c, OPMHIP_ANALYSIS_FAILED, "row %d has %d blocks; the ILU0 tile kernel holds at most %d", i, rows[i + 1] - rows[i], TILE_CAP_BLOCKS);
        if ((rc = alloc_system(c))) return rc;
        c->pattern_set = true;
        return OPMHIP_SUCCESS;
    });
}

int opmhip_upload_system(opmhip_ctx* c, const double* vals, const double* b) {
    if (!c) return OPMHIP_INVALID_ARGUMENT;
    return guarded(c, [&]() -> int {
        if (!c->pattern_set) return fail(c, OPMHIP_NOT_READY, "upload_system before set_pattern");
        OPMHIP_HIP(c, hipSetDevice(c->device));
        int rc = upload_system(c, vals, b);
        if (rc) return rc;
        OPMHIP_HIP(c, hipStreamSynchronize(c->stream));
        return OPMHIP_SUCCESS;
    });
}

int opmhip_solve_system(opmhip_ctx* c, int N, int nnz, int dim, double* vals, const int* rows, const int* cols, const double* b,
                        const opmhip_wells* wells, opmhip_result* res) {
    if (!c) return OPMHIP_INVALID_ARGUMENT;
    return guarded(c, [&]() -> int {
        if (!res) return fail(c, OPMHIP_INVALID_ARGUMENT, "solve_system: res == NULL");
        std::memset(res, 0, sizeof *res);
        if (dim != 3) return fail(c, OPMHIP_INVALID_ARGUMENT, "solve_system: only block size 3 is supported (bda/BdaBridge.cpp:207-211)");
        if (N <= 0 || N % 3 || nnz <= 0 || nnz % 9) return fail(c, OPMHIP_INVALID_ARGUMENT, "solve_system: N/nnz not multiples of the block size");
        OPMHIP_HIP(c, hipSetDevice(c->device));
        const double t0 = now();
        if (!c->pattern_set) {
            if (!rows || !cols) return fail(c, OPMHIP_NOT_READY, "solve_system: first call needs rows/cols");
            int rc = opmhip_set_pattern(c, N / 3, nnz / 9, rows, cols);
            if (rc) return rc == OPMHIP_INVALID_ARGUMENT ? rc : OPMHIP_ANALYSIS_FAILED;
        }
        const Pattern& P = c->pat;
        if (N != P.Nb * 3 || nnz != P.nnzb * 9) return fail(c, OPMHIP_INVALID_ARGUMENT, "solve_system: size differs from the pattern set earlier");
        if (!vals && !c->system_loaded) return fail(c, OPMHIP_NOT_READY, "solve_system: vals == NULL but no matrix is resident on the device");
        if (c->wells.sw.num > 0 && !c->wells.sw.assembled)
            return fail(c, OPMHIP_NOT_READY, "solve_system: a device-resident list of standard wells is set (opmhip_set_std_wells) but not assembled: opmhip_assemble forms its B, C and D^-1");
        int rc;
        if ((rc = upload_system(c, vals, b))) return rc;
        const bool zfix = !vals && c->cfg.zero_diag_fix;
        if ((rc = upload_wells(c, wells))) return rc;
        if (c->wells.sw.num > 0) {
            c->wells.sw.h_flag.resize(c->wells.sw.num);
            OPMHIP_HIP(c, hipMemcpyAsync(c->wells.sw.h_flag.data(), c->wells.sw.flag(), (size_t)c->wells.sw.num * sizeof(double), hipMemcpyDeviceToHost, c->stream));
        }
        OPMHIP_HIP(c, hipStreamSynchronize(c->stream));
        if ((rc = ms_wells_check(c))) return rc;
        std::optional<StdWellsOperatorForm> form;
        if (c->wells.sw.num > 0) {
            if ((rc = std_wells_check(c, c->wells.sw.h_flag.data()))) return rc;
            if (!c->wells.sw.in_matrix) form.emplace(c->wells);
        }
        const double t1 = now();
        FactorRider rider;
        if ((rc = cpr_factor_rider(c, &rider))) return rc;
        launch_ilu_factor(c, zfix, &rider);
        OPMHIP_HIP(c, hipGetLastError());
        OPMHIP_HIP(c, hipStreamSynchronize(c->stream));
        c->factored = true;
        c->cpr.pvals_fresh = rider.mode != 0;
        if (use_cpr(c)) {
            if ((rc = cpr_update(c))) return rc;
            OPMHIP_HIP(c, hipStreamSynchronize(c->stream));
        }
        const double t2 = now();
        if ((rc = bicgstab(c, res))) return rc;
        OPMHIP_HIP(c, hipStreamSynchronize(c->stream));
        const double t3 = now();
        c->have_result = true;
        c->last_solve_iterations = res->iterations;
        res->t_copy = t1 - t0;
        res->t_factor = t2 - t1;
        res->t_solve = t3 - t2;
        res->elapsed = t3 - t0;
        res->num_colors = P.numColors;
        if (c->cfg.verbosity > 0)
            std::fprintf(stderr, "opmhip: converged %d, it %.1f, reduction %.3e, copy %.3f ms, factor %.3f ms, solve %.3f ms\n",
                         res->converged, res->it, res->reduction, 1e3 * res->t_copy, 1e3 * res->t_factor, 1e3 * res->t_solve);
        if (!std::isfinite(res->reduction)) {
            res->converged = 0;
            if (use_cpr(c) && cpr_coarse_pivot_failed(c))
                return fail(c, OPMHIP_CREATE_PRECONDITIONER_FAILED, "CPR: the dense LU of the coarsest pressure level met a zero or non-finite pivot");
            return fail(c, OPMHIP_CREATE_PRECONDITIONER_FAILED, "non-finite residual norm (singular diagonal block in ILU0?)");
        }
        return OPMHIP_SUCCESS;
    });
}

int opmhip_wells_apply_residual(opmhip_ctx* c, const opmhip_wells* wells, const double* res_well) {
    if (!c) return OPMHIP_INVALID_ARGUMENT;
    return guarded(c, [&]() -> int {
        if (!c->system_loaded && !c->asmb.assembled) return fail(c, OPMHIP_NOT_READY, "wells_apply_residual: no residual on the device");
        if (no_standard_wells(c, wells)) return OPMHIP_SUCCESS;
        if (wells->num_wells > 0 && !res_well) return fail(c, OPMHIP_INVALID_ARGUMENT, "wells_apply_residual: null res_well");
        OPMHIP_HIP(c, hipSetDevice(c->device));
        int rc;
        if ((rc = upload_wells(c, wells))) return rc;
        if (wells->num_wells <= 0) return OPMHIP_SUCCESS;
        OPMHIP_HIP(c, hipMemcpyAsync(c->wells.d_res, res_well, (size_t)wells->num_wells * 4 * sizeof(double), hipMemcpyHostToDevice, c->stream));
        launch_wells_residual(c, c->wells.d_res, c->d_b);
        OPMHIP_HIP(c, hipGetLastError());
        OPMHIP_HIP(c, hipStreamSynchronize(c->stream));
        c->wells.num_wells = c->wells.num_ms = 0;
        return OPMHIP_SUCCESS;
    });
}

int opmhip_add_well_contributions(opmhip_ctx* c, const opmhip_wells* wells) {
    if (!c) return OPMHIP_INVALID_ARGUMENT;
    return guarded(c, [&]() -> int {
        if (!c->system_loaded && !c->asmb.assembled) return fail(c, OPMHIP_NOT_READY, "add_well_contributions: no matrix on the device");
        if (wells && wells->distributed != 0 && c->comm.nranks > 1)
            return fail(c, OPMHIP_INVALID_ARGUMENT, "add_well_contributions: a shared list (distributed = 1) cannot be written into the matrix - the blocks that couple "
                                                    "perforations of different subdomains are in no rank's pattern; hand it to opmhip_solve_system instead");
        if (no_standard_wells(c, wells)) return OPMHIP_SUCCESS;
        OPMHIP_HIP(c, hipSetDevice(c->device));
        int rc;
        if ((rc = upload_wells(c, wells))) return rc;
        if (wells->num_wells <= 0) return OPMHIP_SUCCESS;
        const Pattern& P = c->pat;
        const int nw = wells->num_wells;
        std::vector<int> pair_ptr(nw + 1, 0), entry;
        std::vector<char> shares(nw, 0), dup(nw, 0);
        std::unordered_map<int, int> owner;
        for (int w = 0; w < nw; ++w) {
            const int pb = wells->val_pointers[w], np = wells->val_pointers[w + 1] - pb;
            for (int a = 0; a < np; ++a)
                for (int b = 0; b < np; ++b) {
                    const int row = P.toOrder[wells->Ccols[pb + a]], colv = P.toOrder[wells->Bcols[pb + b]];
                    const int* lo = P.col.data() + P.rowptr[row];
                    const int* hi = P.col.data() + P.rowptr[row + 1];
                    const int* it = std::lower_bound(lo, hi, colv);
                    if (it == hi || *it != colv)
                        return fail(c, OPMHIP_INVALID_ARGUMENT, "add_well_contributions: block (%d, %d) of well %d is not in the pattern",
                                    wells->Ccols[pb + a], wells->Bcols[pb + b], w);
                    const int e = (int)(it - P.col.data());
                    entry.push_back(e);
                    auto ins = owner.emplace(e, w);
                    if (!ins.second) {
                        if (ins.first->second != w) shares[w] = 1;
                        else dup[w] = 1;
                    }
                }
            pair_ptr[w + 1] = (int)entry.size();
        }
        struct Scratch {
            int *pp = nullptr, *en = nullptr;
            ~Scratch() { if (pp) (void)hipFree(pp); if (en) (void)hipFree(en); }
        } S;
        OPMHIP_HIP(c, hipMalloc((void**)&S.pp, pair_ptr.size() * sizeof(int)));
        OPMHIP_HIP(c, hipMalloc((void**)&S.en, std::max<size_t>(1, entry.size()) * sizeof(int)));
        OPMHIP_HIP(c, hipMemcpyAsync(S.pp, pair_ptr.data(), pair_ptr.size() * sizeof(int), hipMemcpyHostToDevice, c->stream));
        OPMHIP_HIP(c, hipMemcpyAsync(S.en, entry.data(), entry.size() * sizeof(int), hipMemcpyHostToDevice, c->stream));
        int w0 = 0;
        for (int w = 1; w <= nw; ++w)
            if (w == nw || shares[w] || dup[w] || dup[w - 1]) {
// ... 597 lines not shown
```

opm-autodiff_amd/csrc/capi_asm.cpp:

```cpp
#include <climits>
#include <algorithm>
#include <cmath>
#include <cstring>
#include <map>
#include <string>
#include <vector>

#include "capi_guard.hpp"
#include "fluid_tables.hpp"
#include "internal.hpp"
#include "source_lists.hpp"

using namespace opmhip;

namespace {

template <class T>
std::vector<T> cells_to_internal(const Pattern& P, const T* nat, int width = 1) {
    std::vector<T> v((size_t)P.Nloc * width);
    for (int p = 0; p < P.Nloc; ++p)
        for (int q = 0; q < width; ++q) v[(size_t)p * width + q] = nat[(size_t)P.fromOrder[p] * width + q];
    return v;
}
template <class T>
// ... 395 lines not shown
        OPMHIP_HIP(c, hipMalloc((void**)&S.in, (size_t)4 * n * sizeof(double)));
        OPMHIP_HIP(c, hipMalloc((void**)&S.out, (size_t)8 * n * sizeof(double)));
        const double* src[4] = {p, rs, sw, sg};
        for (int k = 0; k < 4; ++k)
            OPMHIP_HIP(c, hipMemcpyAsync(S.in + (size_t)k * n, src[k], (size_t)n * sizeof(double), hipMemcpyHostToDevice, c->stream));
        launch_fluid_probe(c, pvt_region, sat_region, n, S.in, S.out);
        OPMHIP_HIP(c, hipGetLastError());
        OPMHIP_HIP(c, hipMemcpyAsync(out, S.out, (size_t)8 * n * sizeof(double), hipMemcpyDeviceToHost, c->stream));
        OPMHIP_HIP(c, hipStreamSynchronize(c->stream));
        return OPMHIP_SUCCESS;
    });
}

int opmhip_gas_probe(opmhip_ctx* c, int pvt_region, int n, const double* p, const double* rv, double* out) {
    if (!c) return OPMHIP_INVALID_ARGUMENT;
    return guarded(c, [&]() -> int {
        AsmDev& A = c->asmb;
        if (!A.fluid_set) return fail(c, OPMHIP_NOT_READY, "gas_probe before set_fluid");
        if (n < 0 || (n > 0 && (!p || !rv || !out))) return fail(c, OPMHIP_INVALID_ARGUMENT, "gas_probe: null array");
        if (pvt_region < 0 || pvt_region >= A.num_pvt) return fail(c, OPMHIP_INVALID_ARGUMENT, "gas_probe: region out of range");
        if (n == 0) return OPMHIP_SUCCESS;
        OPMHIP_HIP(c, hipSetDevice(c->device));
        struct Scratch { double *in = nullptr, *out = nullptr; ~Scratch() { if (in) (void)hipFree(in); if (out) (void)hipFree(out); } } S;
        OPMHIP_HIP(c, hipMalloc((void**)&S.in, (size_t)2 * n * sizeof(double)));
        OPMHIP_HIP(c, hipMalloc((void**)&S.out, (size_t)3 * n * sizeof(double)));
        OPMHIP_HIP(c, hipMemcpyAsync(S.in, p, (size_t)n * sizeof(double), hipMemcpyHostToDevice, c->stream));
        OPMHIP_HIP(c, hipMemcpyAsync(S.in + n, rv, (size_t)n * sizeof(double), hipMemcpyHostToDevice, c->stream));
        launch_gas_probe(c, pvt_region, n, S.in, S.out);
        OPMHIP_HIP(c, hipGetLastError());
        OPMHIP_HIP(c, hipMemcpyAsync(out, S.out, (size_t)3 * n * sizeof(double), hipMemcpyDeviceToHost, c->stream));
        OPMHIP_HIP(c, hipStreamSynchronize(c->stream));
        return OPMHIP_SUCCESS;
    });
}

int opmhip_set_state(opmhip_ctx* c, const double* pv, const unsigned char* meaning) {
    if (!c) return OPMHIP_INVALID_ARGUMENT;
    return guarded(c, [&]() -> int {
        if (!c->asmb.static_set) return fail(c, OPMHIP_NOT_READY, "set_state before set_static");
        if (!pv || !meaning) return fail(c, OPMHIP_INVALID_ARGUMENT, "set_state: null array");
        for (int i = 0; i < c->pat.Nloc; ++i)
            if (meaning[i] > (c->asmb.wet_gas ? OPMHIP_SW_PG_RV : OPMHIP_SW_PO_RS))
                return fail(c, OPMHIP_INVALID_ARGUMENT, "set_state: meaning[%d] = %d is not valid (Sw_po_Sg, Sw_po_Rs; Sw_pg_Rv only with a PVTG fluid)", i, (int)meaning[i]);
        OPMHIP_HIP(c, hipSetDevice(c->device));
        AsmDev& A = c->asmb;
        OPMHIP_HIP(c, hipMemcpyAsync(c->d_stageV, pv, (size_t)c->pat.Nloc * 3 * sizeof(double), hipMemcpyHostToDevice, c->stream));
        launch_vec_to_internal(c, c->d_stageV, A.d_pv, c->pat.Nloc);
        OPMHIP_HIP(c, hipMemcpyAsync(A.d_stage_u8, meaning, (size_t)c->pat.Nloc, hipMemcpyHostToDevice, c->stream));
        launch_u8_to_internal(c, A.d_stage_u8, A.d_meaning);
        OPMHIP_HIP(c, hipMemsetAsync(A.d_wasSwitched, 0, c->pat.Nloc, c->stream));
        launch_iq_update(c);
        OPMHIP_HIP(c, hipGetLastError());
        OPMHIP_HIP(c, hipStreamSynchronize(c->stream));
        A.state_set = true;
        A.prev_set = false;
        return OPMHIP_SUCCESS;
    });
}

int opmhip_advance_time_level(opmhip_ctx* c) {
    if (!c) return OPMHIP_INVALID_ARGUMENT;
    return guarded(c, [&]() -> int {
        AsmDev& A = c->asmb;
        if (!A.state_set) return fail(c, OPMHIP_NOT_READY, "advance_time_level before set_state");
        OPMHIP_HIP(c, hipSetDevice(c->device));
        OPMHIP_HIP(c, hipMemcpyAsync(A.d_pv_prev, A.d_pv, (size_t)c->pat.Nloc * 3 * sizeof(double), hipMemcpyDeviceToDevice, c->stream));
        OPMHIP_HIP(c, hipMemcpyAsync(A.d_meaning_prev, A.d_meaning, (size_t)c->pat.Nloc, hipMemcpyDeviceToDevice, c->stream));
        if (int rc = std_wells_save_state(c)) return rc;
        A.prev_set = true;
        return OPMHIP_SUCCESS;
    });
}

int opmhip_relative_change(opmhip_ctx* c, double* relative_change) {
    if (!c || !relative_change) return OPMHIP_INVALID_ARGUMENT;
    return guarded(c, [&]() -> int {
        AsmDev& A = c->asmb;
        if (!A.prev_set) return fail(c, OPMHIP_NOT_READY, "relative_change before advance_time_level: there is no old time level to compare with");
        OPMHIP_HIP(c, hipSetDevice(c->device));
        int rc;
        if (!A.d_rc && (rc = dev_alloc(c, &A.d_rc, (size_t)2 * 256 + 2))) return rc;
        if ((rc = launch_relative_change(c))) return rc;
        double h[2];
        OPMHIP_HIP(c, hipMemcpyAsync(h, A.d_rc + 2 * 256, sizeof(h), hipMemcpyDeviceToHost, c->stream));
        OPMHIP_HIP(c, hipStreamSynchronize(c->stream));
        *relative_change = h[1] > 0.0 ? h[0] / h[1] : 0.0;
        return OPMHIP_SUCCESS;
    });
}

int opmhip_update_failed(opmhip_ctx* c) {
    if (!c) return OPMHIP_INVALID_ARGUMENT;
    return guarded(c, [&]() -> int {
        AsmDev& A = c->asmb;
        if (!A.prev_set) return fail(c, OPMHIP_NOT_READY, "update_failed before advance_time_level");
        OPMHIP_HIP(c, hipSetDevice(c->device));
        OPMHIP_HIP(c, hipMemcpyAsync(A.d_pv, A.d_pv_prev, (size_t)c->pat.Nloc * 3 * sizeof(double), hipMemcpyDeviceToDevice, c->stream));
        OPMHIP_HIP(c, hipMemcpyAsync(A.d_meaning, A.d_meaning_prev, (size_t)c->pat.Nloc, hipMemcpyDeviceToDevice, c->stream));
        OPMHIP_HIP(c, hipMemsetAsync(A.d_wasSwitched, 0, c->pat.Nloc, c->stream));
        launch_iq_update(c);
        OPMHIP_HIP(c, hipGetLastError());
        if (int rc = std_wells_restore_state(c)) return rc;
        A.assembled = false;
        return OPMHIP_SUCCESS;
    });
}

int opmhip_set_composition_change_limits(opmhip_ctx* c, const double* drsdt, const int* drsdt_all, const double* drvdt) {
    if (!c) return OPMHIP_INVALID_ARGUMENT;
    return guarded(c, [&]() -> int {
        AsmDev& A = c->asmb;
        if (!A.state_set) return fail(c, OPMHIP_NOT_READY, "set_composition_change_limits before set_state: lastRs / lastRv are taken from the initial solution");
        if (drvdt && !A.wet_gas) return fail(c, OPMHIP_INVALID_ARGUMENT, "set_composition_change_limits: DRVDT needs a fluid with PVTG");
        OPMHIP_HIP(c, hipSetDevice(c->device));
        OPMHIP_HIP(c, hipStreamSynchronize(c->stream));
        const size_t N = c->pat.Nloc;
        int rc;
        auto put = [&](double** dst, const double* src) -> int {
            if (!*dst && (rc = dev_alloc(c, dst, (size_t)A.num_pvt))) return rc;
            OPMHIP_HIP(c, hipMemcpy(*dst, src, (size_t)A.num_pvt * sizeof(double), hipMemcpyHostToDevice));
            return OPMHIP_SUCCESS;
        };
        A.drsdt_on = drsdt != nullptr;
        A.drvdt_on = drvdt != nullptr;
        if (drsdt) {
            if ((rc = put(&A.d_drsdt, drsdt))) return rc;
            std::vector<int> all(A.num_pvt, 0);
            if (drsdt_all) all.assign(drsdt_all, drsdt_all + A.num_pvt);
            if (!A.d_drsdt_all && (rc = dev_alloc(c, &A.d_drsdt_all, (size_t)A.num_pvt))) return rc;
            OPMHIP_HIP(c, hipMemcpy(A.d_drsdt_all, all.data(), all.size() * sizeof(int), hipMemcpyHostToDevice));
            if (!A.d_lastRs && (rc = dev_alloc(c, &A.d_lastRs, N))) return rc;
            if (!A.d_rsmax && (rc = dev_alloc(c, &A.d_rsmax, N))) return rc;
        } else if (A.d_lastRs) {
            dev_free(c, &A.d_lastRs);
            dev_free(c, &A.d_rsmax);
        }
        if (drvdt) {
            if ((rc = put(&A.d_drvdt, drvdt))) return rc;
            if (!A.d_lastRv && (rc = dev_alloc(c, &A.d_lastRv, N))) return rc;
            if (!A.d_rvmax && (rc = dev_alloc(c, &A.d_rvmax, N))) return rc;
        } else if (A.d_lastRv) {
            dev_free(c, &A.d_lastRv);
            dev_free(c, &A.d_rvmax);
        }
        A.storage_frozen = false;
        if (A.drsdt_on || A.drvdt_on) {
            launch_last_rs_rv(c);
            launch_set_limits(c, 0.0);
        }
        launch_iq_update(c);
        OPMHIP_HIP(c, hipGetLastError());
        OPMHIP_HIP(c, hipStreamSynchronize(c->stream));
        return OPMHIP_SUCCESS;
    });
}

int opmhip_set_irreversible_compaction(opmhip_ctx* c, int enable) {
    if (!c) return OPMHIP_INVALID_ARGUMENT;
    return guarded(c, [&]() -> int {
        AsmDev& A = c->asmb;
        if (!A.state_set) return fail(c, OPMHIP_NOT_READY, "set_irreversible_compaction before set_state: the minimum pressure starts from the initial solution");
        if (enable && A.num_rock <= 0) return fail(c, OPMHIP_INVALID_ARGUMENT, "set_irreversible_compaction: the fluid has no ROCKTAB tables");
        OPMHIP_HIP(c, hipSetDevice(c->device));
        OPMHIP_HIP(c, hipStreamSynchronize(c->stream));
        if (!enable) dev_free(c, &A.d_minpo);
        else {
            int rc;
            if (!A.d_minpo && (rc = dev_alloc(c, &A.d_minpo, (size_t)c->pat.Nloc))) return rc;
// ... 521 lines not shown
        if (Q.num > 0 && dt != Q.step_dt) return fail(c, OPMHIP_INVALID_ARGUMENT, "assemble: dt = %.17g, the aquifers' time step was begun with dt = %.17g", dt, Q.step_dt);
        OPMHIP_HIP(c, hipSetDevice(c->device));
        c->asmb.last_dt = dt;
        c->asmb.last_iteration = iteration;
        SW.in_matrix = false;
        if (SW.num > 0) { launch_std_wells_assemble(c); SW.assembled = true; }
        if (Q.nd > 0) launch_aquifer_apply(c);
        launch_assemble(c, dt, iteration);
        if (Q.nd > 0) launch_aquifer_restore(c);
        if (SW.num > 0) launch_std_wells_restore(c);
        OPMHIP_HIP(c, hipGetLastError());
        c->system_loaded = true;
        c->factored = false;
        c->asmb.assembled = true;
        if (jac) {
            ensure_A(c);
            launch_unpermute_blocks(c, c->d_A, c->d_stageA);
            OPMHIP_HIP(c, hipMemcpyAsync(jac, c->d_stageA, (size_t)c->pat.nnzb * BB * sizeof(double), hipMemcpyDeviceToHost, c->stream));
        }
        if (residual) {
            launch_vec_to_natural(c, c->d_b, c->d_stageV);
            OPMHIP_HIP(c, hipMemcpyAsync(residual, c->d_stageV, (size_t)c->pat.Nb * 3 * sizeof(double), hipMemcpyDeviceToHost, c->stream));
        }
        if (jac || residual) OPMHIP_HIP(c, hipStreamSynchronize(c->stream));
        return OPMHIP_SUCCESS;
    });
}

int opmhip_iq_fields(opmhip_ctx* c) {
    if (!c) return OPMHIP_INVALID_ARGUMENT;
    return iq_doubles_per_cell(c) / 4;
}

int opmhip_get_iq(opmhip_ctx* c, double* out) {
    if (!c) return OPMHIP_INVALID_ARGUMENT;
    return guarded(c, [&]() -> int {
        if (!c->asmb.state_set) return fail(c, OPMHIP_NOT_READY, "get_iq before set_state");
        if (!out) return fail(c, OPMHIP_INVALID_ARGUMENT, "get_iq: out == NULL");
        OPMHIP_HIP(c, hipSetDevice(c->device));
        launch_iq_to_natural(c, c->asmb.d_stage_cell);
        OPMHIP_HIP(c, hipMemcpyAsync(out, c->asmb.d_stage_cell, (size_t)c->pat.Nloc * iq_doubles_per_cell(c) * sizeof(double), hipMemcpyDeviceToHost, c->stream));
        OPMHIP_HIP(c, hipStreamSynchronize(c->stream));
        return OPMHIP_SUCCESS;
    });
}

int opmhip_get_iq_cells(opmhip_ctx* c, int n, const int* cells, double* out) {
    if (!c) return OPMHIP_INVALID_ARGUMENT;
    return guarded(c, [&]() -> int {
        if (!c->asmb.state_set) return fail(c, OPMHIP_NOT_READY, "get_iq_cells before set_state");
        if (n < 0 || (n > 0 && (!cells || !out))) return fail(c, OPMHIP_INVALID_ARGUMENT, "get_iq_cells: n = %d, cells / out missing", n);
        if (n == 0) return OPMHIP_SUCCESS;
        const Pattern& P = c->pat;
        if (n > P.Nloc) return fail(c, OPMHIP_INVALID_ARGUMENT, "get_iq_cells: %d cells asked for, the grid has %d (opmhip_get_iq copies them all)", n, P.Nloc);
        std::vector<int> pos(n);
        for (int i = 0; i < n; ++i) {
            if (cells[i] < 0 || cells[i] >= P.Nloc) return fail(c, OPMHIP_INVALID_ARGUMENT, "get_iq_cells: cell %d of %d", cells[i], P.Nloc);
            pos[i] = P.toOrder[cells[i]];
        }
        OPMHIP_HIP(c, hipSetDevice(c->device));
        const int rc = [&]() -> int {
            int r = stage_cell_positions(c, pos);
            if (r) return r;
            launch_iq_gather(c, n, c->asmb.d_cell_pos, c->asmb.d_stage_cell);
            OPMHIP_HIP(c, hipGetLastError());
            OPMHIP_HIP(c, hipMemcpyAsync(out, c->asmb.d_stage_cell, (size_t)n * iq_doubles_per_cell(c) * sizeof(double), hipMemcpyDeviceToHost, c->stream));
            return OPMHIP_SUCCESS;
        }();
        if (hipStreamSynchronize(c->stream) != hipSuccess && !rc) return fail(c, OPMHIP_DEVICE_ERROR, "get_iq_cells: hipStreamSynchronize failed");
        return rc;
    });
}

int opmhip_convergence(opmhip_ctx* c, double dt, double tol_cnv, double* out) {
    if (!c) return OPMHIP_INVALID_ARGUMENT;
    return guarded(c, [&]() -> int {
        if (!c->asmb.assembled) return fail(c, OPMHIP_NOT_READY, "convergence before assemble");
        if (!out) return fail(c, OPMHIP_INVALID_ARGUMENT, "convergence: out == NULL");
        OPMHIP_HIP(c, hipSetDevice(c->device));
        const int rcc = launch_convergence(c, dt, tol_cnv);
        if (rcc) return rcc;
        OPMHIP_HIP(c, hipGetLastError());
        double h[16];
        OPMHIP_HIP(c, hipMemcpyAsync(h, c->asmb.d_conv_out, 11 * sizeof(double), hipMemcpyDeviceToHost, c->stream));
        OPMHIP_HIP(c, hipStreamSynchronize(c->stream));
        for (int i = 0; i < 11; ++i) out[i] = h[i];
        for (int e = 0; e < 3; ++e) {
            out[11 + e] = h[6 + e] * dt * h[3 + e];
            out[14 + e] = std::fabs(h[6 + e] * h[e]) * dt / h[9];
        }
        return OPMHIP_SUCCESS;
    });
}

int opmhip_reservoir_averages(opmhip_ctx* c, double* out) {
    if (!c) return OPMHIP_INVALID_ARGUMENT;
    return guarded(c, [&]() -> int {
        AsmDev& A = c->asmb;
        if (!A.state_set) return fail(c, OPMHIP_NOT_READY, "reservoir_averages before set_state");
        if (!out) return fail(c, OPMHIP_INVALID_ARGUMENT, "reservoir_averages: out == NULL");
        if (c->comm.nranks > 1 || c->pat.Nghost > 0)
            return fail(c, OPMHIP_INVALID_ARGUMENT, "reservoir_averages: a decomposed context (the sums over the ranks are not formed)");
        OPMHIP_HIP(c, hipSetDevice(c->device));
        int rc;
        if (!A.d_resv && (rc = dev_alloc(c, &A.d_resv, (size_t)RESV_MAX_PARTS * 8 + RESV_OUT))) return rc;
        launch_reservoir_averages(c);
        OPMHIP_HIP(c, hipGetLastError());
        double h[RESV_OUT];
        OPMHIP_HIP(c, hipMemcpyAsync(h, A.d_resv + (size_t)RESV_MAX_PARTS * 8, sizeof(h), hipMemcpyDeviceToHost, c->stream));
        OPMHIP_HIP(c, hipStreamSynchronize(c->stream));
        if (!(h[5] > 0.0)) return fail(c, OPMHIP_INVALID_ARGUMENT, "reservoir_averages: the field's pore volume is %.17g, not > 0", h[5]);
        for (int i = 0; i < 5; ++i) out[i] = h[i];
        return OPMHIP_SUCCESS;
    });
}

int opmhip_update(opmhip_ctx* c, const double* dx, double relax, int* num_switched) {
    if (!c) return OPMHIP_INVALID_ARGUMENT;
    return guarded(c, [&]() -> int {
        if (!c->asmb.state_set) return fail(c, OPMHIP_NOT_READY, "update before set_state");
        if (!dx && !c->have_result) return fail(c, OPMHIP_NOT_READY, "update: dx == NULL but no solve result is resident");
        OPMHIP_HIP(c, hipSetDevice(c->device));
        const double* d_dx = c->d_x;
        if (dx) {
            OPMHIP_HIP(c, hipMemcpyAsync(c->d_stageV, dx, (size_t)c->pat.Nb * 3 * sizeof(double), hipMemcpyHostToDevice, c->stream));
            launch_vec_to_internal(c, c->d_stageV, c->d_t);
            d_dx = c->d_t;
        }
        launch_newton_update(c, d_dx, relax);
        int rcg = launch_ghost_refresh(c);
        if (rcg) return rcg;
        OPMHIP_HIP(c, hipGetLastError());
        if (num_switched) {
            OPMHIP_HIP(c, hipMemcpyAsync(num_switched, c->asmb.d_nswitched, sizeof(int), hipMemcpyDeviceToHost, c->stream));
            OPMHIP_HIP(c, hipStreamSynchronize(c->stream));
        }
        return OPMHIP_SUCCESS;
    });
}

}
```

opm-autodiff_amd/csrc/internal.hpp:

```cpp
#pragma once
#include <hip/hip_runtime.h>

#include <cstdarg>
#include <cstdio>
#include <cstdlib>
#include <cstring>
#include <memory>
#include <climits>
#include <string>
#include <type_traits>
#include <utility>
#include <vector>

#include "../../include/opmhip.h"
#include "cpr_setup.hpp"
#include "vfp_tables.hpp"
#include "source_lists.hpp"

namespace opmhip {

constexpr int BS = 3;
constexpr int BB = 9;

#ifndef OPMHIP_TILE_ROWS
// ... 394 lines not shown
    double* d_pcol = nullptr;
    bool w_given = false;
    double *d_r = nullptr, *d_y = nullptr, *d_z = nullptr;
    double omega = 2.0 / 3.0, damp = 1.6, beta = 0.25;
    CprGatherDev gather;
    int apply_rc = 0;
    bool pvals_fresh = false;
};
struct FactorRider {
    int mode = 0;
    double* w = nullptr;
    double* ap = nullptr;
    double* pcol = nullptr;
    int W = 0;
    int ghostFrom = INT_MAX;
};

enum ProfClass { PROF_SPMV = 0, PROF_ILU_APPLY, PROF_ILU_FACTOR, PROF_VECTOR, PROF_ASSEMBLE, PROF_IQ_UPDATE, PROF_CONVERGENCE, PROF_CPR_AMG,
                 PROF_SPMV_BOUNDARY,
                 PROF_HALO,
                 PROF_ALLREDUCE,
                 PROF_CPR_GATHER,
                 PROF_COUNT };
struct Profiler {
    bool enabled = false;
    int every = 1;
    long solve_no = 0;
    bool suspended = false;
    std::vector<hipEvent_t> ev;
    size_t ev_used = 0;
    std::vector<int> cls, e0, e1;
    size_t used = 0;
    int pending = -1;
    bool lazy = false;
    int handoff = -1;
    static constexpr size_t CAP = 1 << 15;
    double total_ms[PROF_COUNT] = {0};
    long count[PROF_COUNT] = {0};
};

enum Scal {
    SC_RHO = 0, SC_RHOP, SC_ALPHA, SC_OMEGA, SC_BETA, SC_TMP1, SC_TMP2, SC_NORM, SC_NORM0,
    SC_DONE,
    SC_ZERO,
    SC_RR,
    SC_RHOH,
    SC_DONEH,
    SC_COUNT = 16
};

}

struct opmhip_ctx {
    opmhip_config cfg;
    int device = 0;
    hipStream_t stream = nullptr;
    hipEvent_t ev0 = nullptr, ev1 = nullptr;
    std::string err;
    bool pattern_set = false, system_loaded = false, factored = false, have_result = false;
    int ilu_fillin = 0;
    opmhip::Pattern pat;
    double *d_A = nullptr, *d_L = nullptr, *d_U = nullptr, *d_invD = nullptr;
    double *d_R = nullptr, *d_usum = nullptr;
    bool half_product = false;
    bool split_asm = false;
    bool A_stale = false;
    long long split_gathers = 0, split_assemblies = 0;
    double *d_b = nullptr, *d_x = nullptr, *d_r = nullptr, *d_rw = nullptr, *d_p = nullptr, *d_v = nullptr,
           *d_s = nullptr, *d_t = nullptr, *d_pw = nullptr, *d_vu = nullptr;
    double *d_stageA = nullptr, *d_stageV = nullptr;
    double* d_scal = nullptr;
    double* d_part = nullptr;
    double minv_scale = 1.0;
    double* d_part2 = nullptr;
    int npart = 0;
    int last_solve_iterations = 0;
    int last_dot_count = 0;
    double* h_pinned = nullptr;
    static constexpr int RB_SLOTS = 4, RB_DOUBLES = 4;
    double* h_ring = nullptr;
    double* d_ring = nullptr;
    double rb_seq = 0.0;
    double rb_want[RB_SLOTS] = {0, 0, 0, 0};
    const double* d_done = nullptr;
    opmhip::WellsDev wells;
    opmhip::AsmDev asmb;
    opmhip::CommDev comm;
    opmhip::CprDev cpr;
    opmhip::Profiler prof;
    std::vector<void*> allocs;
    struct HostRange { const void* p; size_t bytes; };
    std::vector<HostRange> pinned;
};

namespace opmhip {

inline const char* tuning_env(const char* name) {
    static const bool on = [] { const char* e = std::getenv("OPMHIP_TUNING"); return e && e[0] == '1'; }();
    const char* v = std::getenv(name);
    if (!v) return nullptr;
    if (!on) {
        std::fprintf(stderr, "opmhip: %s is set but OPMHIP_TUNING=1 is not - ignored\n", name);
        return nullptr;
    }
    std::fprintf(stderr, "opmhip: measurement switch %s=%s is in force\n", name, v);
    return v;
}

inline int fail(opmhip_ctx* c, int code, const char* fmt, ...) {
    char buf[512];
    va_list ap;
    va_start(ap, fmt);
    vsnprintf(buf, sizeof buf, fmt, ap);
    va_end(ap);
    if (c) c->err = buf;
    return code;
}

#define OPMHIP_HIP(ctx, call)                                                                       \
    do {                                                                                            \
        hipError_t e_ = (call);                                                                     \
        if (e_ != hipSuccess)                                                                       \
            return opmhip::fail(ctx, OPMHIP_DEVICE_ERROR, "%s failed: %s (%s:%d)", #call,           \
                                hipGetErrorString(e_), __FILE__, __LINE__);                         \
    } while (0)

inline bool poison_allocations() {
    static const bool on = [] { const char* e = tuning_env("OPMHIP_POISON_ALLOC"); return e && e[0] == '1'; }();
    return on;
}
template <class T>
int dev_alloc(opmhip_ctx* c, T** p, size_t count) {
    void* q = nullptr;
    size_t bytes = (count ? count : 1) * sizeof(T);
    hipError_t e = hipMalloc(&q, bytes);
    if (e != hipSuccess)
        return fail(c, OPMHIP_DEVICE_ERROR, "hipMalloc(%zu) failed: %s", bytes, hipGetErrorString(e));
    if (poison_allocations() && ((e = hipMemset(q, std::is_floating_point<T>::value ? 0xFF : 0x00, bytes)) != hipSuccess || (e = hipDeviceSynchronize()) != hipSuccess)) {
        (void)hipFree(q);
        return fail(c, OPMHIP_DEVICE_ERROR, "hipMemset(%zu) failed: %s", bytes, hipGetErrorString(e));
    }
    c->allocs.push_back(q);
    *p = static_cast<T*>(q);
    return OPMHIP_SUCCESS;
}
template <class T>
void dev_free(opmhip_ctx* c, T** p) {
    if (!*p) return;
    for (size_t i = 0; i < c->allocs.size(); ++i)
        if (c->allocs[i] == (void*)*p) { c->allocs[i] = c->allocs.back(); c->allocs.pop_back(); break; }
    (void)hipFree((void*)*p);
    *p = nullptr;
}
template <class P>
void dev_part_release(opmhip_ctx* c, P& part) {
    part.each_dev([c](auto** p) { dev_free(c, p); });
    part = P();
}
template <class P>
void dev_part_install(opmhip_ctx* c, P& in_force, P& fresh) {
    dev_part_release(c, in_force);
    in_force = std::move(fresh);
}
template <class T>
int dev_upload(opmhip_ctx* c, T** p, const std::vector<T>& h) {
    int rc = dev_alloc(c, p, h.size());
    if (rc) return rc;
    if (!h.empty()) OPMHIP_HIP(c, hipMemcpy(*p, h.data(), h.size() * sizeof(T), hipMemcpyHostToDevice));
    return OPMHIP_SUCCESS;
}

inline int prof_event(opmhip_ctx* c, hipStream_t s = nullptr) {
    Profiler& P = c->prof;
    if (P.ev.size() <= P.ev_used) {
        hipEvent_t e;
        if (hipEventCreate(&e) != hipSuccess) return -1;
        P.ev.push_back(e);
    }
    const int i = (int)P.ev_used++;
    (void)hipEventRecord(P.ev[i], s ? s : c->stream);
    return i;
}
inline int prof_event_slot(opmhip_ctx* c) {
    Profiler& P = c->prof;
    if (P.ev.size() <= P.ev_used) {
        hipEvent_t e;
        if (hipEventCreate(&e) != hipSuccess) return -1;
        P.ev.push_back(e);
    }
    return (int)P.ev_used++;
}
inline void prof_flush(opmhip_ctx* c) {
    Profiler& P = c->prof;
    P.handoff = -1;
    if (P.pending < 0) return;
    const int e = prof_event(c);
    if (e >= 0) P.e1[P.pending] = e; else P.cls[P.pending] = -1;
    P.pending = -1;
}
inline int prof_begin(opmhip_ctx* c, int cls) {
    Profiler& P = c->prof;
    if (!P.enabled || P.suspended || P.used >= Profiler::CAP) { prof_flush(c); return -1; }
    int e;
    if (P.handoff >= 0) { e = P.handoff; P.handoff = -1; }
    else e = prof_event(c);
    if (e < 0) return -1;
    if (P.pending >= 0) { P.e1[P.pending] = e; P.pending = -1; }
    if (P.cls.size() <= P.used) { P.cls.push_back(cls); P.e0.push_back(e); P.e1.push_back(-1); }
    const int slot = (int)P.used++;
    P.cls[slot] = cls; P.e0[slot] = e; P.e1[slot] = -1;
    return slot;
}
inline bool prof_kernel_scope(opmhip_ctx* c, int cls, int* es, int* ee) {
    Profiler& P = c->prof;
    if (!P.enabled || P.suspended || P.used >= Profiler::CAP) return false;
    *es = prof_event_slot(c);
    *ee = prof_event_slot(c);
    if (*es < 0 || *ee < 0) return false;
    if (P.pending >= 0) { P.e1[P.pending] = *es; P.pending = -1; }
    if (P.cls.size() <= P.used) { P.cls.push_back(cls); P.e0.push_back(*es); P.e1.push_back(*ee); }
    const int slot = (int)P.used++;
    P.cls[slot] = cls; P.e0[slot] = *es; P.e1[slot] = *ee;
    P.handoff = P.lazy ? *ee : -1;
    return true;
}
inline void prof_end(opmhip_ctx* c, int slot) {
    if (slot < 0) return;
    c->prof.pending = slot;
    if (!c->prof.lazy) prof_flush(c);
}
inline int prof_span_begin(opmhip_ctx* c, int cls, hipStream_t s = nullptr) {
    Profiler& P = c->prof;
    if (!P.enabled || P.suspended || P.used >= Profiler::CAP) return -1;
    const int e = prof_event(c, s);
    if (e < 0) return -1;
    if (P.cls.size() <= P.used) { P.cls.push_back(cls); P.e0.push_back(e); P.e1.push_back(-1); }
    const int slot = (int)P.used++;
    P.cls[slot] = cls; P.e0[slot] = e; P.e1[slot] = -1;
    return slot;
}
inline void prof_span_end(opmhip_ctx* c, int slot, hipStream_t s = nullptr) {
    if (slot < 0) return;
    const int e = prof_event(c, s);
    if (e >= 0) c->prof.e1[slot] = e; else c->prof.cls[slot] = -1;
}

int build_pattern(opmhip_ctx* c, int Nb, int Nghost, int nnzb, const int* rows, const int* cols);

void launch_permute_blocks(opmhip_ctx* c, const double* nat, double* internal);
void launch_unpermute_blocks(opmhip_ctx* c, const double* internal, double* nat);
void launch_vec_to_internal(opmhip_ctx* c, const double* nat, double* internal, int cells = -1);
void launch_vec_to_natural(opmhip_ctx* c, const double* internal, double* nat, int cells = -1);
void launch_zero_diag_fix(opmhip_ctx* c);
int launch_spmv(opmhip_ctx* c, double* x, double* y, int ndot, const double* w0, double xs = 1.0, bool exchange = false, const double* uadd = nullptr, const double* w1 = nullptr);
bool split_asm_wanted(const opmhip_ctx* c);
void ensure_A(opmhip_ctx* c);
bool half_product_wanted(const opmhip_ctx* c);
void launch_wells_residual(opmhip_ctx* c, const double* d_resWell, double* r);
void launch_wells_add_to_matrix(opmhip_ctx* c, int w0, int nw, int serial, const int* d_pair_ptr, const int* d_entry);
int launch_wells_recover(opmhip_ctx* c, const double* d_resWell, const double* x, double* d_xw);
void launch_ilu_factor(opmhip_ctx* c, bool fix_zero_diagonal = false, const FactorRider* rider = nullptr);
int cpr_factor_rider(opmhip_ctx* c, FactorRider* r);
void launch_ilu_apply(opmhip_ctx* c, const double* d, double* v, double w_override = -1.0, double* unscaled = nullptr, const double* addp = nullptr, double* work = nullptr, double* usum = nullptr);
int cpr_update(opmhip_ctx* c, bool solveBoundary = true);
void launch_cpr_apply(opmhip_ctx* c, const double* d, double* v);
int cpr_set_weights(opmhip_ctx* c, const double* w);
int cpr_level_sizes(const opmhip_ctx* c, int* n, int* nnz, int cap);
void cpr_shutdown(opmhip_ctx* c);
bool cpr_coarse_pivot_failed(opmhip_ctx* c);
int cpr_ilu_levels_in_force(const opmhip_ctx* c);
inline bool use_cpr(const opmhip_ctx* c) { return c->cfg.preconditioner == OPMHIP_PRECOND_CPR_QUASIIMPES || c->cfg.preconditioner == OPMHIP_PRECOND_CPR_TRUEIMPES; }
void ms_wells_tree_plan(opmhip_ctx* c, const std::vector<MsTreeDesc>& tdesc);
void launch_ms_wells_factor(opmhip_ctx* c);
int launch_wells_apply(opmhip_ctx* c, const double* x, double* y, double xs = 1.0);
void launch_lu_to_natural(opmhip_ctx* c, double* d_out_internal_layout);
int bicgstab(opmhip_ctx* c, opmhip_result* res);
int comm_allreduce(opmhip_ctx* c, double* d_buf, int n, int op );
int comm_allgather(opmhip_ctx* c, const double* d_send, double* d_recv, size_t count);
int comm_halo_f64(opmhip_ctx* c, double* vec, int w, hipStream_t s = nullptr);
int comm_halo_begin(opmhip_ctx* c, double* vec);
int comm_halo_end(opmhip_ctx* c);
int comm_halo_u8(opmhip_ctx* c, unsigned char* vec);
void comm_halo_bystander(opmhip_ctx* c);
void comm_release(opmhip_ctx* c);
void launch_iq_update(opmhip_ctx* c);
int launch_ghost_refresh(opmhip_ctx* c);
void launch_newton_update(opmhip_ctx* c, const double* d_dx_internal, double relax);
void launch_assemble(opmhip_ctx* c, double dt, int iteration);
void launch_drift_update(opmhip_ctx* c, double dt);
void launch_aquifer_begin(opmhip_ctx* c);
void launch_aquifer_apply(opmhip_ctx* c);
void launch_aquifer_restore(opmhip_ctx* c);
void launch_aquifer_end(opmhip_ctx* c, double dt);
int std_wells_check(opmhip_ctx* c, const double* flags);
int std_wells_save_state(opmhip_ctx* c);
int std_wells_restore_state(opmhip_ctx* c);
void launch_std_wells_solve(opmhip_ctx* c, bool first);
void launch_std_wells_wellbore(opmhip_ctx* c, bool first, bool init);
void launch_std_wells_controls(opmhip_ctx* c);
void launch_std_wells_groups(opmhip_ctx* c, int iteration, bool check);
void launch_std_wells_resv(opmhip_ctx* c);
void launch_std_wells_assemble(opmhip_ctx* c);
void launch_std_wells_restore(opmhip_ctx* c);
void launch_std_wells_axpy(opmhip_ctx* c, double relax);
void launch_std_wells_add_to_matrix(opmhip_ctx* c);
void launch_last_rs_rv(opmhip_ctx* c);
void launch_set_limits(opmhip_ctx* c, double dt);
void launch_min_pressure(opmhip_ctx* c, bool init);
void launch_storage_old(opmhip_ctx* c);
void launch_max_oil_saturation(opmhip_ctx* c, bool init);
void launch_max_water_saturation(opmhip_ctx* c, bool init);
void launch_hyst_update(opmhip_ctx* c, const double* d_sw_ow = nullptr, const double* d_sw_go = nullptr);
int launch_relative_change(opmhip_ctx* c);
int launch_convergence(opmhip_ctx* c, double dt, double tol_cnv);
void launch_reservoir_averages(opmhip_ctx* c);
double* resv_avg_kernels(opmhip_ctx* c);
void launch_u8_to_internal(opmhip_ctx* c, const unsigned char* nat, unsigned char* internal);
void launch_u8_to_natural(opmhip_ctx* c, const unsigned char* internal, unsigned char* nat);
void launch_iq_to_natural(opmhip_ctx* c, double* d_nat);
void launch_iq_gather(opmhip_ctx* c, int n, const int* d_pos, double* d_out);
void launch_source_scatter(opmhip_ctx* c, int n, const int* d_pos, const double* d_src, const double* d_dsrc);
int iq_doubles_per_cell(const opmhip_ctx* c);
int asm_max_rows();
int launch_fluid_probe(opmhip_ctx* c, int pr, int sr, int n, const double* d_in, double* d_out);
int launch_vfp_probe(opmhip_ctx* c, int table, int n, const double* d_in, bool has_target, double* d_out);
int launch_gas_probe(opmhip_ctx* c, int pr, int n, const double* d_in, double* d_out);
int launch_sat_probe(opmhip_ctx* c, int sr, int cfg, const double* d_eps, int n, const double* d_in, double* d_out);
int asm_threads();
void launch_vector_kernels_once(opmhip_ctx* c);
void launch_stream_read(opmhip_ctx* c);

}
```

opm-autodiff_amd/csrc/solver.hip:

```cpp
#include <hip/hip_runtime.h>
#include <hip/hip_ext.h>
#include <atomic>

#include <chrono>
#include <climits>
#include <cmath>
#include <cstdlib>

#include "device_blocks.hpp"
#include "internal.hpp"
#include "ms_wells_setup.hpp"

namespace opmhip {

#ifndef OPMHIP_STAGE_DEPTH
#define OPMHIP_STAGE_DEPTH 16
#endif
typedef double v2d_t __attribute__((ext_vector_type(2)));
__device__ __forceinline__ double2 ld_stream(const double2* p) {
    const v2d_t t = __builtin_nontemporal_load(reinterpret_cast<const v2d_t*>(p));
    return make_double2(t.x, t.y);
}
__device__ __forceinline__ void st_rowsum(double* p, double v) {
    __builtin_nontemporal_store(v, p);
// ... 2608 lines not shown
        return OPMHIP_SUCCESS;
    }
    hipLaunchKernelGGL(k_finalize3, dim3(1), dim3(VB), 0, c->stream, mode, count, c->d_part, c->npart, c->d_scal, tol, hslot, seq, (double)rb_half);
    return OPMHIP_SUCCESS;
}
void launch_vector_kernels_once(opmhip_ctx* c) {
    const int n = c->pat.Nb * BS, nb = vec_blocks(n);
    hipLaunchKernelGGL(k_bicg_pupdate, dim3(nb), dim3(VB), 0, c->stream, n, c->d_scal, c->d_p, c->d_v, c->d_r);
    hipLaunchKernelGGL(k_bicg_upd1<false>, dim3(nb), dim3(VB), 0, c->stream, n, c->d_scal, c->d_r, c->d_v, c->d_part, c->npart, -1.0);
    (void)finalize(c, FIN_NORM, nb);
    hipLaunchKernelGGL(k_bicg_upd2<false>, dim3(nb), dim3(VB), 0, c->stream, n, c->d_scal, c->d_x, c->d_pw, c->d_s, c->d_r, c->d_t, c->d_rw, c->d_part, c->npart, c->minv_scale, -1.0);
    (void)finalize(c, FIN_NORM_RHO, nb);
}

static int read_scalars(opmhip_ctx* c) {
    OPMHIP_HIP(c, hipMemcpyAsync(c->h_pinned, c->d_scal, SC_COUNT * sizeof(double), hipMemcpyDeviceToHost, c->stream));
    OPMHIP_HIP(c, hipStreamSynchronize(c->stream));
    return OPMHIP_SUCCESS;
}
enum { HALF_ALL = 0, HALF_PRECOND = 1, HALF_REST = 2 };
static int enqueue_half(opmhip_ctx* c, int h, int part = HALF_ALL) {
    const Pattern& P = c->pat;
    const int n = P.Nb * BS, nb = vec_blocks(n);
    const bool cpr = use_cpr(c);
    const bool hp = !cpr && c->half_product;
    const bool sr = c->cfg.fused_reductions > 0;
    const bool precTalks = cpr && c->cpr.gather.on;
    const bool head = part != HALF_REST, rest = part != HALF_PRECOND;
    const bool applyNow = part == HALF_ALL || (precTalks ? part == HALF_REST : part == HALF_PRECOND);
    int rc, ps;
    if ((h & 1) == 0) {
        if (head && h > 0) {
            ps = prof_begin(c, PROF_VECTOR);
            hipLaunchKernelGGL(k_bicg_pupdate, dim3(nb), dim3(VB), 0, c->stream, n, c->d_scal, c->d_p, c->d_v, c->d_r);
            prof_end(c, ps);
        }
        if (applyNow) {
            if (cpr) launch_cpr_apply(c, c->d_p, c->d_pw);
            else launch_ilu_apply(c, c->d_p, c->d_pw, -1.0, &c->minv_scale, nullptr, nullptr, hp ? c->d_usum : nullptr);
            if (cpr && c->cpr.apply_rc) { rc = c->cpr.apply_rc; c->cpr.apply_rc = 0; return rc; }
        }
        if (!rest) return OPMHIP_SUCCESS;
        if (sr) {
            if ((rc = launch_spmv(c, c->d_pw, c->d_v, 3, c->d_rw, c->minv_scale, true, hp ? c->d_usum : nullptr, c->d_r))) return rc;
            ps = prof_begin(c, PROF_VECTOR);
            if ((rc = finalize3(c, FIN_SR1, dot_count(c), h))) return rc;
            hipLaunchKernelGGL(k_bicg_upd1<true>, dim3(nb), dim3(VB), 0, c->stream, n, c->d_scal, c->d_r, c->d_v, c->d_part, c->npart, (double)h);
            prof_end(c, ps);
            return OPMHIP_SUCCESS;
        }
        if ((rc = launch_spmv(c, c->d_pw, c->d_v, 1, c->d_rw, c->minv_scale, true, hp ? c->d_usum : nullptr))) return rc;
        ps = prof_begin(c, PROF_VECTOR);
        if ((rc = finalize(c, FIN_ALPHA, dot_count(c)))) return rc;
        hipLaunchKernelGGL(k_bicg_upd1<false>, dim3(nb), dim3(VB), 0, c->stream, n, c->d_scal, c->d_r, c->d_v, c->d_part, c->npart, -1.0);
        if ((rc = finalize(c, FIN_NORM, nb, h))) return rc;
        prof_end(c, ps);
    } else {
        if (applyNow) {
            if (cpr) launch_cpr_apply(c, c->d_r, c->d_s);
            else launch_ilu_apply(c, c->d_r, c->d_s, -1.0, &c->minv_scale, nullptr, nullptr, hp ? c->d_usum : nullptr);
            if (cpr && c->cpr.apply_rc) { rc = c->cpr.apply_rc; c->cpr.apply_rc = 0; return rc; }
        }
        if (!rest) return OPMHIP_SUCCESS;
        if (sr) {
            if ((rc = launch_spmv(c, c->d_s, c->d_t, 3, c->d_r, c->minv_scale, true, hp ? c->d_usum : nullptr, c->d_rw))) return rc;
            ps = prof_begin(c, PROF_VECTOR);
            if ((rc = finalize3(c, FIN_SR2, dot_count(c), h))) return rc;
            hipLaunchKernelGGL(k_bicg_upd2<true>, dim3(nb), dim3(VB), 0, c->stream, n, c->d_scal, c->d_x, c->d_pw, c->d_s, c->d_r, c->d_t, c->d_rw, c->d_part, c->npart, c->minv_scale, (double)h);
            prof_end(c, ps);
            return OPMHIP_SUCCESS;
        }
        if ((rc = launch_spmv(c, c->d_s, c->d_t, 2, c->d_r, c->minv_scale, true, hp ? c->d_usum : nullptr))) return rc;
        ps = prof_begin(c, PROF_VECTOR);
        if ((rc = finalize(c, FIN_OMEGA, dot_count(c)))) return rc;
        hipLaunchKernelGGL(k_bicg_upd2<false>, dim3(nb), dim3(VB), 0, c->stream, n, c->d_scal, c->d_x, c->d_pw, c->d_s, c->d_r, c->d_t, c->d_rw, c->d_part, c->npart, c->minv_scale, -1.0);
        if ((rc = finalize(c, FIN_NORM_RHO, nb, h))) return rc;
        prof_end(c, ps);
    }
    return OPMHIP_SUCCESS;
}
static int wait_half(opmhip_ctx* c, int h, double* norm, double* norm_0) {
    const int sl = h % opmhip_ctx::RB_SLOTS;
    const volatile double* slot = c->h_ring + (size_t)sl * opmhip_ctx::RB_DOUBLES;
    const double want = c->rb_want[sl];
    const auto t0 = std::chrono::steady_clock::now();
    for (unsigned long spin = 1;; ++spin) {
        if (slot[3] == want) break;
        if ((spin & 0xFFFFu) == 0) {
            const hipError_t e = hipStreamQuery(c->stream);
            if (e == hipSuccess) {
                if (slot[3] == want) break;
                return fail(c, OPMHIP_DEVICE_ERROR, "BiCGStab: the stream drained without the stopping-rule record of half iteration %d", h);
            }
            if (e != hipErrorNotReady) return fail(c, OPMHIP_DEVICE_ERROR, "BiCGStab: %s", hipGetErrorString(e));
            if (std::chrono::steady_clock::now() - t0 > std::chrono::seconds(120))
                return fail(c, OPMHIP_DEVICE_ERROR, "BiCGStab: no stopping-rule record of half iteration %d after 120 s", h);
        }
#if defined(__x86_64__) || defined(__i386__)
        __builtin_ia32_pause();
#elif defined(__aarch64__)
        asm volatile("yield" ::: "memory");
#endif
    }
    std::atomic_thread_fence(std::memory_order_acquire);
    *norm = slot[0];
    *norm_0 = slot[1];
    return OPMHIP_SUCCESS;
}
int bicgstab(opmhip_ctx* c, opmhip_result* res) {
    const Pattern& P = c->pat;
    const int n = P.Nb * BS, nb = vec_blocks(n);
    const int maxit = c->cfg.maxit;
    const double tol = c->cfg.tolerance;
    struct SolveScope {
        opmhip_ctx* c;
        explicit SolveScope(opmhip_ctx* c_) : c(c_) {
            c->d_done = c->d_scal + SC_DONE;
            Profiler& Q = c->prof;
            Q.solve_no += 1;
            Q.suspended = Q.enabled && Q.every > 1 && (Q.solve_no % Q.every) != 0;
            Q.lazy = c->comm.nranks == 1;
        }
        ~SolveScope() {
            c->d_done = c->d_scal + SC_ZERO;
            c->prof.lazy = false;
            prof_flush(c);
            c->prof.suspended = false;
        }
    } scope(c);
    int rc;
    c->minv_scale = 1.0;
    hipLaunchKernelGGL(k_bicg_init, dim3(nb), dim3(VB), 0, c->stream, n, c->d_b, c->d_r, c->d_rw, c->d_p, c->d_x, c->d_v, c->d_part, c->npart);
    if ((rc = finalize(c, FIN_INIT, nb))) return rc;
    const int nhalves = 2 * maxit;
    double norm = 0.0, norm_0 = 0.0;
    float it = maxit + 0.5f;
    size_t mark_next = c->prof.used;
    const bool split = c->comm.nranks > 1;
    if (nhalves > 0 && (rc = enqueue_half(c, 0))) return rc;
    for (int h = 0; h < nhalves; ++h) {
        mark_next = c->prof.used;
        if (h + 1 < nhalves && (rc = enqueue_half(c, h + 1, split ? HALF_PRECOND : HALF_ALL))) return rc;
        if ((rc = wait_half(c, h, &norm, &norm_0))) return rc;
        if (!std::isfinite(norm)) {
            prof_flush(c);
            break;
        }
        if (norm < tol * norm_0) {
            it = 0.5f * (float)(h + 1);
            prof_flush(c);
            for (size_t i = mark_next; i < c->prof.used; ++i) c->prof.cls[i] = -1;
            if ((h & 1) == 0) hipLaunchKernelGGL(k_bicg_xhalf, dim3(nb), dim3(VB), 0, c->stream, n, c->d_scal, c->d_x, c->d_pw, c->minv_scale);
            break;
        }
        if (split && h + 1 < nhalves && (rc = enqueue_half(c, h + 1, HALF_REST))) return rc;
    }
    if (nhalves <= 0) {
        if ((rc = read_scalars(c))) return rc;
        norm = norm_0 = c->h_pinned[SC_NORM0];
    }
    bool drifted = false;
    if (c->cfg.fused_reductions > 0 && nhalves > 0 && std::isfinite(norm)) {
        hipLaunchKernelGGL(k_dots, dim3(nb), dim3(VB), 0, c->stream, n, c->d_r, c->d_r, c->d_part, c->npart, 1);
        if ((rc = finalize(c, FIN_TRUE, nb))) return rc;
        if ((rc = read_scalars(c))) return rc;
        const double truth = c->h_pinned[SC_TMP1];
        drifted = it != (maxit + 0.5f) && !(truth < 2.0 * tol * norm_0);
        norm = truth;
    }
    OPMHIP_HIP(c, hipGetLastError());
    res->it = it;
    res->iterations = (int)std::fmin(it, (float)maxit);
    res->reduction = norm / norm_0;
    res->conv_rate = std::pow(res->reduction, 1.0 / it);
    res->converged = (it != (maxit + 0.5f)) && !drifted;
    return OPMHIP_SUCCESS;
}

}
```

opm-autodiff_amd/newton.py:

```python
import time
from dataclasses import dataclass, field


class NumericalIssue(RuntimeError):
    pass


class TooManyIterations(RuntimeError):
    pass


@dataclass
class SimulatorReportSingle:
    assemble_time: float = 0.0
    linear_solve_setup_time: float = 0.0
    linear_solve_time: float = 0.0
    update_time: float = 0.0
    total_linearizations: int = 0
    total_newton_iterations: int = 0
    total_linear_iterations: int = 0
    converged: bool = False

    def __iadd__(self, o):
        for k in ("assemble_time", "linear_solve_setup_time", "linear_solve_time", "update_time", "total_linearizations",
# ... 58 lines not shown
        if it < 2:
            return False
        F0, F1, F2 = h[it], h[it - 1], h[it - 2]
        osc = 0
        for p in range(3):
            d1 = abs((F0[p] - F2[p]) / F0[p])
            d2 = abs((F0[p] - F1[p]) / F0[p])
            osc += (d1 < self.param.relax_rel_tol) and (self.param.relax_rel_tol < d2)
        return osc > 1

    def nonlinear_iteration(self, iteration, dt):
        rep = SimulatorReportSingle()
        if iteration == 0:
            self.residual_norms_history = []
            self.current_relaxation = 1.0
        rep.total_linearizations = 1
        t0 = time.perf_counter()
        wa = None
        dev_wells = self.wells is not None and getattr(self.wells, "on_device", False)
        if dev_wells:
            if self.aquifers is not None and not self.aquifers.on_device:
                raise NotImplementedError("HostAquifers beside DeviceStandardWells: the influx would replace the caller's source rows behind the wells' back")
            self.wells.begin_iteration(iteration)
        elif self.wells is not None:
            iq = self.wells.records(self.m)
            if iteration == 0:
                self.wells.calculate_explicit_quantities(iq)
                self.wells.solve_well_equations(iq)
            if getattr(self.wells, "groups", None):
                self.wells.update_well_controls(iteration)
            else:
                self.wells.update_well_controls()
            host_aq = self.aquifers is not None and not self.aquifers.on_device
            if hasattr(self.m, "set_source_cells"):
                wa = self.wells.assemble(iq)
                if not host_aq:
                    self.m.set_source_cells(wa["cells"], wa["source_cells"], wa["dsource_cells"])
            else:
                wa = self.wells.assemble(iq, iq.shape[0])
                self.m.set_source(wa["source"], wa["dsource"])
                if host_aq:
                    raise NotImplementedError("HostAquifers beside a well model needs a model object with set_source_cells")
        if self.aquifers is not None and not self.aquifers.on_device:
            if wa is not None:
                self.aquifers.add_to_source(self.m, wa["cells"], wa["source_cells"], wa["dsource_cells"])
            else:
                self.aquifers.add_to_source(self.m)
        self.m.assemble(dt, iteration, fetch=False)
        conv, norms = self.get_convergence(dt, iteration)
        if wa is not None:
            conv = conv and self.wells.converged(wa["res_well"])
        if dev_wells:
            self.wells.fetch()
            conv = conv and self.wells.converged()
        t1 = time.perf_counter()
        rep.assemble_time += t1 - t0
        rep.converged = conv and iteration > self.param.newton_min_iter
        self.residual_norms_history.append(norms)
        if not rep.converged:
            rep.total_newton_iterations = 1
            if wa is not None:
                self.m.wells_apply_residual(wa["wells"], wa["res_well"])
                res = self.m.solve_jacobian_system(wells=wa["wells"])
            elif dev_wells:
                self.m.std_wells_apply_residual()
                if self.wells.matrix_add:
                    self.m.std_wells_add_to_matrix()
                res = self.m.solve_jacobian_system()
            else:
                res = self.m.solve_jacobian_system()
            rep.linear_solve_setup_time += res.t_factor
            rep.linear_solve_time += res.t_solve + res.t_copy
            rep.total_linear_iterations += res.iterations
            self.last_linear_iterations = res.iterations
            if not res.converged:
                raise NumericalIssue("Convergence failure for linear solver.")
            t2 = time.perf_counter()
            if self.param.use_update_stabilization and self.detect_oscillations(iteration):
                self.current_relaxation = max(self.current_relaxation - self.param.relax_increment, self.param.relax_max)
            if wa is not None:
                self.wells.update(self.m.wells_recover_solution(wa["wells"], wa["res_well"]), self.current_relaxation)
            if dev_wells:
                self.wells.update(self.current_relaxation)
            self.m.update(None, self.current_relaxation)
            rep.update_time += time.perf_counter() - t2
        return rep

    def step(self, dt):
        report = SimulatorReportSingle()
        iteration = 0
        converged = False
        while True:
            it_rep = self.nonlinear_iteration(iteration, dt)
            report += it_rep
            converged = it_rep.converged
            iteration += 1
            if not ((not converged and iteration <= self.param.newton_max_iter) or iteration <= self.param.newton_min_iter):
                break
        if not converged:
            raise TooManyIterations("Failed to complete a time step within %d iterations." % self.param.newton_max_iter)
        report.converged = True
        return report

    def advance_time_level(self):
        self.m.advance_time_level()
        if self.wells is not None and not getattr(self.wells, "on_device", False):
            self._well_saved = self.wells.state()

    def update_failed(self):
        self.m.update_failed()
        if self.wells is not None and self._well_saved is not None:
            self.wells.set_state(self._well_saved)

    def relative_change(self):
        return self.m.relative_change() if hasattr(self.m, "relative_change") else None

    def begin_time_step(self, dt, time=0.0):
        if hasattr(self.m, "begin_time_step"):
            self.m.begin_time_step(dt)
        if self.aquifers is not None:
            self.aquifers.begin_time_step(self.m, time, dt)

    def end_time_step(self, dt):
        self.m.end_time_step(dt)
        if self.aquifers is not None and not self.aquifers.on_device:
            self.aquifers.end_time_step(dt)


@dataclass
class TimeSteppingParameters:
    restart_factor: float = 0.33
    growth_factor: float = 2.0
    max_growth: float = 3.0
    max_restarts: int = 10
    target_newton_iterations: int = 8
    decay_damping: float = 1.0
    growth_damping: float = 3.2
    time_step_control: str = "pid+newtoniteration"
    time_step_control_tolerance: float = 1e-1
    min_time_step_based_on_newton_iterations: float = 0.0
    initial_dt: float = 86400.0
    max_dt: float = 365.0 * 86400.0


class PIDTimeStepControl:

    def __init__(self, tol):
        self.tol = float(tol)
        self.errors = [self.tol] * 3

    def compute(self, dt, error):
        import numpy as np
        e = self.errors
        e[0], e[1] = e[1], e[2]
        e[2] = float(error)
        tol = self.tol
        if error > tol:
            return dt * tol / error
        kP, kI, kD = 0.075, 0.175, 0.01
        with np.errstate(divide="ignore", invalid="ignore", over="ignore"):
            e0, e1, e2 = (np.float64(v) for v in e)
            return float(dt * np.power(e1 / e2, kP) * np.power(tol / e2, kI) * np.power(e0 * e0 / e1 / e2, kD))


class AdaptiveTimeStepping:

    def __init__(self, model, param=None):
# ... 92 lines not shown
```

Before: 86.00.

## Replace per-stage stream syncs with mapped host records and lean solve path

Per-stage scalar results (convergence norms, relative change, switch count) are now published by the final reduction kernel into pinned mapped host memory with a release-store sequence word. The host spin-waits on that word instead of issuing a memcpy plus full stream synchronize. The solve path drops its intermediate stream synchronizations in the simple single-rank ILU case and times the factorization with events. The Newton update skips counting and reading back switched cells when the caller doesn't need the count. This cuts host-device round trips and launch-queue bubbles per Newton iteration, at the cost of host busy-polling and an env/API toggle to restore the old behaviour.

Result: no change. 86.15 (median of 2 runs) (+0.2%).

```diff
diff --git a/include/opmhip.h b/include/opmhip.h
--- a/include/opmhip.h
+++ b/include/opmhip.h
@@ -122,6 +122,8 @@
 const char* opmhip_last_error(const opmhip_ctx* ctx);
 int opmhip_abi_version(void);
 int opmhip_synchronize(opmhip_ctx* ctx);
+int opmhip_set_stage_sync(opmhip_ctx* ctx, int on);
+int opmhip_get_stage_sync(opmhip_ctx* ctx, int* on);
 
 int opmhip_set_pattern(opmhip_ctx* ctx, int Nb, int nnzb, const int* rows, const int* cols);
 int opmhip_set_pattern_dd(opmhip_ctx* ctx, int Nb, int Nghost, int nnzb, const int* rows, const int* cols);
diff --git a/opm-autodiff_amd/capi.py b/opm-autodiff_amd/capi.py
--- a/opm-autodiff_amd/capi.py
+++ b/opm-autodiff_amd/capi.py
@@ -364,6 +364,8 @@
         L.opmhip_profile_enable.argtypes = [vp, C.c_int]
         L.opmhip_profile_get.argtypes = [vp, C.c_int, C.POINTER(C.c_longlong), C.POINTER(C.c_double)]
         L.opmhip_synchronize.argtypes = [vp]
+        L.opmhip_set_stage_sync.argtypes = [vp, C.c_int]
+        L.opmhip_get_stage_sync.argtypes = [vp, C.POINTER(C.c_int)]
         L.opmhip_comm_info.argtypes = [vp, ip]
         L.opmhip_comm_selftest.argtypes = [vp, dp]
         L.opmhip_set_vfp_tables.argtypes = [vp, C.POINTER(VfpTables)]
@@ -650,6 +652,14 @@
 
     def synchronize(self):
         self._check(lib().opmhip_synchronize(self._h))
+
+    def set_stage_sync(self, on):
+        self._check(lib().opmhip_set_stage_sync(self._h, int(bool(on))))
+
+    def stage_sync(self):
+        on = C.c_int(0)
+        self._check(lib().opmhip_get_stage_sync(self._h, C.byref(on)))
+        return bool(on.value)
 
     def comm_info(self):
         a = np.zeros(4, np.int32)
@@ -1191,3 +1201,6 @@
         n = C.c_int(0)
         self._check(lib().opmhip_update(self._h, _ptr(dx), relax, C.byref(n)))
         return n.value
+
+    def update_resident(self, relax=1.0):
+        self._check(lib().opmhip_update(self._h, None, relax, None))
diff --git a/opm-autodiff_amd/csrc/assemble.hip b/opm-autodiff_amd/csrc/assemble.hip
--- a/opm-autodiff_amd/csrc/assemble.hip
+++ b/opm-autodiff_amd/csrc/assemble.hip
@@ -538,7 +538,7 @@
     wasSwitched[c] = sw ? 1 : 0;
     meaning[c] = (unsigned char)mng;
     pv[(size_t)c * 3] = x[0]; pv[(size_t)c * 3 + 1] = x[1]; pv[(size_t)c * 3 + 2] = x[2];
-    if (sw) atomicAdd(nswitched, 1);
+    if (sw && nswitched) atomicAdd(nswitched, 1);
     Iq<Ad> q;
     update_iq<Ad, DP, EXT>(T, C, c, x, mng, q);
     store_iq<EXT>(iq, C.ncell, c, q);
@@ -1004,7 +1004,7 @@
     __syncthreads();
     if (threadIdx.x == 0) part[blockIdx.x] = sh[0] + sh[1] + sh[2] + sh[3];
 }
-__global__ __launch_bounds__(256) void k_conv_final2(int nblocks, const double* __restrict__ part, double* __restrict__ out) {
+__global__ __launch_bounds__(256) void k_conv_final2(int nblocks, const double* __restrict__ part, double* __restrict__ out, double* rec, double seq) {
     __shared__ double sh[256];
     double a = 0.0;
     for (int b = threadIdx.x; b < nblocks; b += 256) a += part[b];
@@ -1014,7 +1014,14 @@
         if ((int)threadIdx.x < o) sh[threadIdx.x] += sh[threadIdx.x + o];
         __syncthreads();
     }
-    if (threadIdx.x == 0) out[10] = sh[0];
+    if (threadIdx.x == 0) {
+        out[10] = sh[0];
+        if (rec) {
+            for (int i = 0; i < 10; ++i) rec[i] = out[i];
+            rec[10] = sh[0];
+            record_publish(rec + opmhip_ctx::Record::CAP, seq);
+        }
+    }
 }
 
 constexpr int RESV_SUMS = 8;
@@ -1324,15 +1331,16 @@
         hipLaunchKernelGGL(k_iq_update<true>, dim3(cdiv(Nloc - Nb, 256)), dim3(256), 0, c->stream, Nb, Nloc, tables_of(c), cells_of(c), c->asmb.d_pv, c->asmb.d_meaning, c->asmb.d_iq));
     return OPMHIP_SUCCESS;
 }
-void launch_newton_update(opmhip_ctx* c, const double* d_dx, double relax) {
+void launch_newton_update(opmhip_ctx* c, const double* d_dx, double relax, bool count) {
     const int Nb = c->pat.Nb;
-    (void)hipMemsetAsync(c->asmb.d_nswitched, 0, sizeof(int), c->stream);
+    int* nswitched = count ? c->asmb.d_nswitched : nullptr;
+    if (count) (void)hipMemsetAsync(nswitched, 0, sizeof(int), c->stream);
     const int ps = prof_begin(c, PROF_IQ_UPDATE);
     OPMHIP_LAYOUT(c,
         hipLaunchKernelGGL(k_newton_update<false>, dim3(cdiv(Nb, 256)), dim3(256), 0, c->stream, Nb, tables_of(c), cells_of(c), d_dx, relax, c->asmb.d_pv,
-                           c->asmb.d_meaning, c->asmb.d_wasSwitched, c->asmb.d_iq, c->asmb.d_nswitched),
+                           c->asmb.d_meaning, c->asmb.d_wasSwitched, c->asmb.d_iq, nswitched),
         hipLaunchKernelGGL(k_newton_update<true>, dim3(cdiv(Nb, 256)), dim3(256), 0, c->stream, Nb, tables_of(c), cells_of(c), d_dx, relax, c->asmb.d_pv,
-                           c->asmb.d_meaning, c->asmb.d_wasSwitched, c->asmb.d_iq, c->asmb.d_nswitched));
+                           c->asmb.d_meaning, c->asmb.d_wasSwitched, c->asmb.d_iq, nswitched));
     prof_end(c, ps);
 }
 void launch_assemble(opmhip_ctx* c, double dt, int iteration) {
@@ -1422,24 +1430,50 @@
     }
     if (threadIdx.x == 0) { part[blockIdx.x] = sd[0]; part[RC_PARTS + blockIdx.x] = sn[0]; }
 }
-__global__ __launch_bounds__(64) void k_relative_change_final(const double* __restrict__ part, double* __restrict__ out) {
+__global__ __launch_bounds__(64) void k_relative_change_final(const double* __restrict__ part, double* __restrict__ out, double* rec, double seq) {
     if (threadIdx.x != 0) return;
     double d = 0.0, q = 0.0;
     for (int i = 0; i < RC_PARTS; ++i) { d += part[i]; q += part[RC_PARTS + i]; }
     out[0] = d; out[1] = q;
+    if (rec) {
+        rec[0] = d; rec[1] = q;
+        record_publish(rec + opmhip_ctx::Record::CAP, seq);
+    }
+}
+__global__ void k_update_record(const int* __restrict__ nswitched, double* rec, double seq) {
+    rec[0] = (double)nswitched[0];
+    record_publish(rec + opmhip_ctx::Record::CAP, seq);
 }
 int launch_relative_change(opmhip_ctx* c) {
     const AsmDev& A = c->asmb;
     double* part = A.d_rc;
     double* out = A.d_rc + 2 * RC_PARTS;
     hipLaunchKernelGGL(k_relative_change_part, dim3(RC_PARTS), dim3(256), 0, c->stream, c->pat.Nb, A.d_pv, A.d_meaning, A.d_pv_prev, A.d_meaning_prev, part);
-    hipLaunchKernelGGL(k_relative_change_final, dim3(1), dim3(64), 0, c->stream, part, out);
+    double* rec = nullptr;
+    double seq = 0.0;
+    if (stage_records(c)) {
+        if (int rc = record_next(c, &c->rec_rc, &seq)) return rc;
+        rec = c->rec_rc.d;
+    }
+    hipLaunchKernelGGL(k_relative_change_final, dim3(1), dim3(64), 0, c->stream, part, out, rec, seq);
     if (c->comm.nranks > 1) return comm_allreduce(c, out, 2, 0);
     return OPMHIP_SUCCESS;
 }
+int launch_update_record(opmhip_ctx* c) {
+    double seq = 0.0;
+    if (int rc = record_next(c, &c->rec_upd, &seq)) return rc;
+    hipLaunchKernelGGL(k_update_record, dim3(1), dim3(1), 0, c->stream, c->asmb.d_nswitched, c->rec_upd.d, seq);
+    return OPMHIP_SUCCESS;
+}
 
 int launch_convergence(opmhip_ctx* c, double dt, double tol_cnv) {
     const int Nb = c->pat.Nb, nb = cdiv(Nb, 256);
+    double* rec = nullptr;
+    double seq = 0.0;
+    if (stage_records(c)) {
+        if (int rc = record_next(c, &c->rec_conv, &seq)) return rc;
+        rec = c->rec_conv.d;
+    }
     const int ps = prof_begin(c, PROF_CONVERGENCE);
     hipLaunchKernelGGL(k_conv_pass1, dim3(nb), dim3(256), 0, c->stream, Nb, cells_of(c), c->d_b, c->asmb.d_conv_part);
     const bool dd = c->comm.nranks > 1;
@@ -1452,7 +1486,7 @@
         hipLaunchKernelGGL(k_conv_unpack, dim3(1), dim3(64), 0, c->stream, c->comm.d_red, (double)c->comm.global_cells, c->asmb.d_conv_out);
     }
     hipLaunchKernelGGL(k_conv_pass2, dim3(nb), dim3(256), 0, c->stream, Nb, cells_of(c), c->d_b, c->asmb.d_conv_out, dt, tol_cnv, c->asmb.d_conv_part);
-    hipLaunchKernelGGL(k_conv_final2, dim3(1), dim3(256), 0, c->stream, nb, c->asmb.d_conv_part, c->asmb.d_conv_out);
+    hipLaunchKernelGGL(k_conv_final2, dim3(1), dim3(256), 0, c->stream, nb, c->asmb.d_conv_part, c->asmb.d_conv_out, rec, seq);
     if (dd) {
         const int rc = comm_allreduce(c, c->asmb.d_conv_out + 10, 1, 0);
         if (rc) return rc;
diff --git a/opm-autodiff_amd/csrc/capi.cpp b/opm-autodiff_amd/csrc/capi.cpp
--- a/opm-autodiff_amd/csrc/capi.cpp
+++ b/opm-autodiff_amd/csrc/capi.cpp
@@ -1,4 +1,5 @@
 #include <cstdlib>
+#include <atomic>
 #include <chrono>
 #include <unordered_map>
 #include <algorithm>
@@ -11,6 +12,48 @@
 #include "ms_wells_setup.hpp"
 
 using namespace opmhip;
+
+namespace opmhip {
+int record_wait(opmhip_ctx* c, const volatile double* seq_word, double want, const char* what) {
+    const auto t0 = std::chrono::steady_clock::now();
+    for (unsigned long spin = 1;; ++spin) {
+        if (*seq_word == want) break;
+        if ((spin & 0xFFFFu) == 0) {
+            const hipError_t e = hipStreamQuery(c->stream);
+            if (e == hipSuccess) {
+                if (*seq_word == want) break;
+                return fail(c, OPMHIP_DEVICE_ERROR, "%s: the stream drained without the record", what);
+            }
+            if (e != hipErrorNotReady) return fail(c, OPMHIP_DEVICE_ERROR, "%s: %s", what, hipGetErrorString(e));
+            if (std::chrono::steady_clock::now() - t0 > std::chrono::seconds(120))
+                return fail(c, OPMHIP_DEVICE_ERROR, "%s: no record after 120 s", what);
+        }
+#if defined(__x86_64__) || defined(__i386__)
+        __builtin_ia32_pause();
+#elif defined(__aarch64__)
+        asm volatile("yield" ::: "memory");
+#endif
+    }
+    std::atomic_thread_fence(std::memory_order_acquire);
+    return OPMHIP_SUCCESS;
+}
+int record_next(opmhip_ctx* c, opmhip_ctx::Record* r, double* seq) {
+    if (!r->h) {
+        constexpr size_t bytes = (opmhip_ctx::Record::CAP + 1) * sizeof(double);
+        double* h = nullptr;
+        OPMHIP_HIP(c, hipHostMalloc((void**)&h, bytes, hipHostMallocMapped));
+        std::memset(h, 0, bytes);
+        const hipError_t e = hipHostGetDevicePointer((void**)&r->d, h, 0);
+        if (e != hipSuccess) {
+            (void)hipHostFree(h);
+            return fail(c, OPMHIP_DEVICE_ERROR, "hipHostGetDevicePointer failed: %s", hipGetErrorString(e));
+        }
+        r->h = h;
+    }
+    *seq = (r->seq += 1.0);
+    return OPMHIP_SUCCESS;
+}
+}
 
 namespace {
 thread_local std::string g_err = "";
@@ -339,6 +382,8 @@
         delete c;
         return OPMHIP_DEVICE_ERROR;
     }
+    static const bool stage_sync = [] { const char* v = tuning_env("OPMHIP_STAGE_SYNC"); return v && v[0] == '1'; }();
+    c->stage_sync = stage_sync ? 1 : 0;
     *out = c;
     return OPMHIP_SUCCESS;
 }
@@ -357,6 +402,8 @@
     if (c->wells.h_y) (void)hipHostFree(c->wells.h_y);
     if (c->wells.ms.h_flag) (void)hipHostFree(c->wells.ms.h_flag);
     if (c->h_ring) (void)hipHostFree(c->h_ring);
+    for (opmhip_ctx::Record* r : {&c->rec_conv, &c->rec_rc, &c->rec_upd})
+        if (r->h) (void)hipHostFree(r->h);
     if (c->asmb.aq.h_step) (void)hipHostFree(c->asmb.aq.h_step);
     if (c->asmb.aq.ev_step) (void)hipEventDestroy(c->asmb.aq.ev_step);
     if (c->ev0) (void)hipEventDestroy(c->ev0);
@@ -375,6 +422,20 @@
     return OPMHIP_SUCCESS;
 }
 
+int opmhip_set_stage_sync(opmhip_ctx* c, int on) {
+    if (!c) return OPMHIP_INVALID_ARGUMENT;
+    if (on != 0 && on != 1) return fail(c, OPMHIP_INVALID_ARGUMENT, "set_stage_sync: on must be 0 or 1");
+    c->stage_sync = on;
+    return OPMHIP_SUCCESS;
+}
+
+int opmhip_get_stage_sync(opmhip_ctx* c, int* on) {
+    if (!c) return OPMHIP_INVALID_ARGUMENT;
+    if (!on) return fail(c, OPMHIP_INVALID_ARGUMENT, "get_stage_sync: on == NULL");
+    *on = c->stage_sync;
+    return OPMHIP_SUCCESS;
+}
+
 int opmhip_set_pattern(opmhip_ctx* c, int Nb, int nnzb, const int* rows, const int* cols) {
     return opmhip_set_pattern_dd(c, Nb, 0, nnzb, rows, cols);
 }
@@ -428,6 +489,8 @@
         if (c->wells.sw.num > 0 && !c->wells.sw.assembled)
             return fail(c, OPMHIP_NOT_READY, "solve_system: a device-resident list of standard wells is set (opmhip_set_std_wells) but not assembled: opmhip_assemble forms its B, C and D^-1");
         int rc;
+        const bool lean = !c->stage_sync && !vals && !b && !wells && c->comm.nranks == 1 && !use_cpr(c) && !c->cfg.fused_reductions &&
+                          c->wells.sw.num == 0 && c->wells.ms.num == 0 && !c->wells.ms.flag_pending;
         if ((rc = upload_system(c, vals, b))) return rc;
         const bool zfix = !vals && c->cfg.zero_diag_fix;
         if ((rc = upload_wells(c, wells))) return rc;
@@ -435,7 +498,7 @@
             c->wells.sw.h_flag.resize(c->wells.sw.num);
             OPMHIP_HIP(c, hipMemcpyAsync(c->wells.sw.h_flag.data(), c->wells.sw.flag(), (size_t)c->wells.sw.num * sizeof(double), hipMemcpyDeviceToHost, c->stream));
         }
-        OPMHIP_HIP(c, hipStreamSynchronize(c->stream));
+        if (!lean) OPMHIP_HIP(c, hipStreamSynchronize(c->stream));
         if ((rc = ms_wells_check(c))) return rc;
         std::optional<StdWellsOperatorForm> form;
         if (c->wells.sw.num > 0) {
@@ -445,9 +508,11 @@
         const double t1 = now();
         FactorRider rider;
         if ((rc = cpr_factor_rider(c, &rider))) return rc;
+        if (lean) OPMHIP_HIP(c, hipEventRecord(c->ev0, c->stream));
         launch_ilu_factor(c, zfix, &rider);
         OPMHIP_HIP(c, hipGetLastError());
-        OPMHIP_HIP(c, hipStreamSynchronize(c->stream));
+        if (lean) OPMHIP_HIP(c, hipEventRecord(c->ev1, c->stream));
+        else OPMHIP_HIP(c, hipStreamSynchronize(c->stream));
         c->factored = true;
         c->cpr.pvals_fresh = rider.mode != 0;
         if (use_cpr(c)) {
@@ -456,13 +521,20 @@
         }
         const double t2 = now();
         if ((rc = bicgstab(c, res))) return rc;
-        OPMHIP_HIP(c, hipStreamSynchronize(c->stream));
+        if (!lean) OPMHIP_HIP(c, hipStreamSynchronize(c->stream));
         const double t3 = now();
         c->have_result = true;
         c->last_solve_iterations = res->iterations;
         res->t_copy = t1 - t0;
         res->t_factor = t2 - t1;
         res->t_solve = t3 - t2;
+        if (lean) {
+            float ms = 0.0f;
+            OPMHIP_HIP(c, hipEventSynchronize(c->ev1));
+            OPMHIP_HIP(c, hipEventElapsedTime(&ms, c->ev0, c->ev1));
+            res->t_factor = 1e-3 * (double)ms;
+            if (t3 - t1 > res->t_factor) res->t_solve = (t3 - t1) - res->t_factor;
+        }
         res->elapsed = t3 - t0;
         res->num_colors = P.numColors;
         if (c->cfg.verbosity > 0)
diff --git a/opm-autodiff_amd/csrc/capi_asm.cpp b/opm-autodiff_amd/csrc/capi_asm.cpp
--- a/opm-autodiff_amd/csrc/capi_asm.cpp
+++ b/opm-autodiff_amd/csrc/capi_asm.cpp
@@ -501,8 +501,13 @@
         if (!A.d_rc && (rc = dev_alloc(c, &A.d_rc, (size_t)2 * 256 + 2))) return rc;
         if ((rc = launch_relative_change(c))) return rc;
         double h[2];
-        OPMHIP_HIP(c, hipMemcpyAsync(h, A.d_rc + 2 * 256, sizeof(h), hipMemcpyDeviceToHost, c->stream));
-        OPMHIP_HIP(c, hipStreamSynchronize(c->stream));
+        if (stage_records(c)) {
+            if ((rc = record_wait(c, c->rec_rc, "relative_change"))) return rc;
+            h[0] = c->rec_rc.h[0]; h[1] = c->rec_rc.h[1];
+        } else {
+            OPMHIP_HIP(c, hipMemcpyAsync(h, A.d_rc + 2 * 256, sizeof(h), hipMemcpyDeviceToHost, c->stream));
+            OPMHIP_HIP(c, hipStreamSynchronize(c->stream));
+        }
         *relative_change = h[1] > 0.0 ? h[0] / h[1] : 0.0;
         return OPMHIP_SUCCESS;
     });
@@ -1190,8 +1195,13 @@
         if (rcc) return rcc;
         OPMHIP_HIP(c, hipGetLastError());
         double h[16];
-        OPMHIP_HIP(c, hipMemcpyAsync(h, c->asmb.d_conv_out, 11 * sizeof(double), hipMemcpyDeviceToHost, c->stream));
-        OPMHIP_HIP(c, hipStreamSynchronize(c->stream));
+        if (stage_records(c)) {
+            if (int rc = record_wait(c, c->rec_conv, "convergence")) return rc;
+            for (int i = 0; i < 11; ++i) h[i] = c->rec_conv.h[i];
+        } else {
+            OPMHIP_HIP(c, hipMemcpyAsync(h, c->asmb.d_conv_out, 11 * sizeof(double), hipMemcpyDeviceToHost, c->stream));
+            OPMHIP_HIP(c, hipStreamSynchronize(c->stream));
+        }
         for (int i = 0; i < 11; ++i) out[i] = h[i];
         for (int e = 0; e < 3; ++e) {
             out[11 + e] = h[6 + e] * dt * h[3 + e];
@@ -1235,11 +1245,18 @@
             launch_vec_to_internal(c, c->d_stageV, c->d_t);
             d_dx = c->d_t;
         }
-        launch_newton_update(c, d_dx, relax);
+        int discarded = 0;
+        if (!num_switched && c->stage_sync) num_switched = &discarded;
+        launch_newton_update(c, d_dx, relax, num_switched != nullptr);
         int rcg = launch_ghost_refresh(c);
         if (rcg) return rcg;
         OPMHIP_HIP(c, hipGetLastError());
-        if (num_switched) {
+        if (num_switched && stage_records(c)) {
+            if (int rc = launch_update_record(c)) return rc;
+            OPMHIP_HIP(c, hipGetLastError());
+            if (int rc = record_wait(c, c->rec_upd, "update")) return rc;
+            *num_switched = (int)c->rec_upd.h[0];
+        } else if (num_switched) {
             OPMHIP_HIP(c, hipMemcpyAsync(num_switched, c->asmb.d_nswitched, sizeof(int), hipMemcpyDeviceToHost, c->stream));
             OPMHIP_HIP(c, hipStreamSynchronize(c->stream));
         }
diff --git a/opm-autodiff_amd/csrc/internal.hpp b/opm-autodiff_amd/csrc/internal.hpp
--- a/opm-autodiff_amd/csrc/internal.hpp
+++ b/opm-autodiff_amd/csrc/internal.hpp
@@ -500,6 +500,14 @@
     double* d_ring = nullptr;
     double rb_seq = 0.0;
     double rb_want[RB_SLOTS] = {0, 0, 0, 0};
+    struct Record {
+        static constexpr int CAP = 12;
+        double* h = nullptr;
+        double* d = nullptr;
+        double seq = 0.0;
+    };
+    Record rec_conv, rec_rc, rec_upd;
+    int stage_sync = 0;
     const double* d_done = nullptr;
     opmhip::WellsDev wells;
     opmhip::AsmDev asmb;
@@ -542,6 +550,15 @@
             return opmhip::fail(ctx, OPMHIP_DEVICE_ERROR, "%s failed: %s (%s:%d)", #call,           \
                                 hipGetErrorString(e_), __FILE__, __LINE__);                         \
     } while (0)
+
+int record_wait(opmhip_ctx* c, const volatile double* seq_word, double want, const char* what);
+int record_next(opmhip_ctx* c, opmhip_ctx::Record* r, double* seq);
+inline int record_wait(opmhip_ctx* c, const opmhip_ctx::Record& r, const char* what) { return record_wait(c, r.h + opmhip_ctx::Record::CAP, r.seq, what); }
+#if defined(__HIPCC__)
+__device__ __forceinline__ void record_publish(double* seq_word, double seq) {
+    __hip_atomic_store(seq_word, seq, __ATOMIC_RELEASE, __HIP_MEMORY_SCOPE_SYSTEM);
+}
+#endif
 
 inline bool poison_allocations() {
     static const bool on = [] { const char* e = tuning_env("OPMHIP_POISON_ALLOC"); return e && e[0] == '1'; }();
@@ -703,7 +720,9 @@
 void comm_release(opmhip_ctx* c);
 void launch_iq_update(opmhip_ctx* c);
 int launch_ghost_refresh(opmhip_ctx* c);
-void launch_newton_update(opmhip_ctx* c, const double* d_dx_internal, double relax);
+inline bool stage_records(const opmhip_ctx* c) { return !c->stage_sync && c->comm.nranks == 1; }
+void launch_newton_update(opmhip_ctx* c, const double* d_dx_internal, double relax, bool count = true);
+int launch_update_record(opmhip_ctx* c);
 void launch_assemble(opmhip_ctx* c, double dt, int iteration);
 void launch_drift_update(opmhip_ctx* c, double dt);
 void launch_aquifer_begin(opmhip_ctx* c);
diff --git a/opm-autodiff_amd/csrc/solver.hip b/opm-autodiff_amd/csrc/solver.hip
--- a/opm-autodiff_amd/csrc/solver.hip
+++ b/opm-autodiff_amd/csrc/solver.hip
@@ -2714,25 +2714,10 @@
 static int wait_half(opmhip_ctx* c, int h, double* norm, double* norm_0) {
     const int sl = h % opmhip_ctx::RB_SLOTS;
     const volatile double* slot = c->h_ring + (size_t)sl * opmhip_ctx::RB_DOUBLES;
-    const double want = c->rb_want[sl];
-    const auto t0 = std::chrono::steady_clock::now();
-    for (unsigned long spin = 1;; ++spin) {
-        if (slot[3] == want) break;
-        if ((spin & 0xFFFFu) == 0) {
-            const hipError_t e = hipStreamQuery(c->stream);
-            if (e == hipSuccess) {
-                if (slot[3] == want) break;
-                return fail(c, OPMHIP_DEVICE_ERROR, "BiCGStab: the stream drained without the stopping-rule record of half iteration %d", h);
-            }
-            if (e != hipErrorNotReady) return fail(c, OPMHIP_DEVICE_ERROR, "BiCGStab: %s", hipGetErrorString(e));
-            if (std::chrono::steady_clock::now() - t0 > std::chrono::seconds(120))
-                return fail(c, OPMHIP_DEVICE_ERROR, "BiCGStab: no stopping-rule record of half iteration %d after 120 s", h);
-        }
-#if defined(__x86_64__) || defined(__i386__)
-        __builtin_ia32_pause();
-#elif defined(__aarch64__)
-        asm volatile("yield" ::: "memory");
-#endif
+    if (slot[3] != c->rb_want[sl]) {
+        char what[64];
+        std::snprintf(what, sizeof what, "BiCGStab: stopping-rule record of half iteration %d", h);
+        if (int rc = record_wait(c, slot + 3, c->rb_want[sl], what)) return rc;
     }
     std::atomic_thread_fence(std::memory_order_acquire);
     *norm = slot[0];
diff --git a/opm-autodiff_amd/newton.py b/opm-autodiff_amd/newton.py
--- a/opm-autodiff_amd/newton.py
+++ b/opm-autodiff_amd/newton.py
@@ -164,7 +164,10 @@
                 self.wells.update(self.m.wells_recover_solution(wa["wells"], wa["res_well"]), self.current_relaxation)
             if dev_wells:
                 self.wells.update(self.current_relaxation)
-            self.m.update(None, self.current_relaxation)
+            if hasattr(self.m, "update_resident"):
+                self.m.update_resident(self.current_relaxation)
+            else:
+                self.m.update(None, self.current_relaxation)
             rep.update_time += time.perf_counter() - t2
         return rep
 
```
